# eblerjana/pangenie

Measured on AMD Instinct MI355X. Metric: genotyped variants/sec (whole node) at H haplotypes; HBM GB/s vs roofline, higher is better.
Workload: dtype f64

## Files before the change

include/pangenie_hmm.h:

```cpp
#ifndef PANGENIE_HMM_H
#define PANGENIE_HMM_H

#include <stddef.h>
#include <stdint.h>

#ifdef __cplusplus
extern "C" {
#endif

#define PG_OK 0
#define PG_ERR_INVALID (-1)
#define PG_ERR_NO_PATHS (-2)
#define PG_ERR_UNSUPPORTED (-3)
#define PG_ERR_DEVICE (-4)
#define PG_ERR_NOMEM (-5)

typedef struct pg_contig_batch {
    uint32_t n_variants;
    uint32_t n_paths;
    const uint64_t* variant_pos;
    const uint16_t* coverage;
    const uint32_t* kmer_off;
    const uint16_t* kmer_count;
    const uint32_t* allele_off;
    const uint16_t* allele_id;
    const uint8_t*  allele_flags;
    const uint16_t* allele_kmer_off;
    const uint32_t* allele_kmer_mask;
    const uint16_t* path_allele;
} pg_contig_batch;

typedef struct pg_hmm_params {
    long double effective_N;
    double recombrate;
    int32_t uniform;
    int32_t run_genotyping;
    int32_t run_phasing;
    int32_t reserved;
} pg_hmm_params;
#define PG_CALL_ANNOUNCED 1

typedef struct pg_contig_result {
    double*   lik;
    int32_t*  lik_exp;
    uint8_t*  kept;
    uint8_t*  allele_present;
    uint16_t* n_kmers;
    uint16_t* coverage;
    uint32_t  n_columns;
    uint32_t  reserved;
    uint16_t* haplotype_1;
    uint16_t* haplotype_2;
} pg_contig_result;

int pg_hmm_geno_offsets(const pg_contig_batch* batch, uint64_t* geno_off);

typedef struct pg_table pg_table;
pg_table* pg_table_create(uint16_t cov_min, uint16_t cov_max, uint16_t count_max,
                          long double regularization);
pg_table* pg_table_create_default(void);
int  pg_table_modify(pg_table* t, uint16_t coverage, uint16_t count,
                     long double p0, long double p1, long double p2);
int  pg_table_get(const pg_table* t, uint16_t coverage, uint16_t count,
                  long double out3[3]);
void pg_table_destroy(pg_table* t);

int pg_hmm_device_count(void);
const char* pg_hmm_version(void);
int pg_hmm_genotype_contig(const pg_contig_batch* batch, const pg_table* table,
                           const pg_hmm_params* params, int device,
                           pg_contig_result* out, char* err, size_t errlen);
void pg_hmm_announce(int device);
void pg_hmm_retract(int device);
int  pg_hmm_coalesce_stats(uint64_t out3[3]);

typedef struct pg_job pg_job;
pg_job* pg_job_create(int device, uint32_t n_contigs, const pg_contig_batch* batches,
                      const pg_table* table, const pg_hmm_params* params,
                      char* err, size_t errlen);
int  pg_job_run(pg_job* job, void* stream, char* err, size_t errlen);
int  pg_job_fetch(pg_job* job, uint32_t contig, pg_contig_result* out, char* err, size_t errlen);
int  pg_job_fetch_all(pg_job* job, pg_contig_result* outs, char* err, size_t errlen);
int  pg_job_device_results(pg_job* job, uint32_t contig, void** d_lik, uint64_t* n_lik,
                           void** d_lik_exp, uint64_t* n_variants);
#define PG_N_KERNEL_CLASSES 6
int  pg_job_kernel_ms(const pg_job* job, double ms[PG_N_KERNEL_CLASSES]);
const char* pg_job_kernel_name(int cls);
int  pg_job_profile_counters(pg_job* job, uint32_t contig, uint64_t out64[64]);
uint64_t pg_job_device_bytes(const pg_job* job);
int  pg_job_sweep_mode(const pg_job* job, uint32_t* chunk_cols);
uint32_t pg_job_triangle_chains(const pg_job* job);
double pg_job_index_ms(const pg_job* job);
size_t pg_job_plan(const pg_job* job, char* out, size_t len);
int pg_sparse_segment(uint32_t n_columns, uint32_t chunk_cols, uint32_t chunk, uint32_t role, uint32_t j, uint32_t out[3]);
int pg_sparse_stored_by_chain(uint32_t n_columns, uint32_t role, uint32_t column);
int pg_sparse_chunk_segment(uint32_t n_columns, uint32_t chunk_cols, uint32_t chunk, uint32_t role, uint32_t j, uint32_t out[3]);
int pg_sparse_chunk_stored_by_chain(uint32_t n_columns, uint32_t role, uint32_t column);
int pg_sparse_piece_range(uint32_t n_columns, uint32_t chunk_cols, uint32_t piece_chunks, uint32_t piece, uint32_t role, uint32_t out[2]);
double pg_job_viterbi_ms(const pg_job* job);
void pg_job_destroy(pg_job* job);

int  pg_job_panel_sizes(const pg_job* job, uint32_t contig, uint32_t* n_variants, uint32_t* n_paths,
                        uint64_t* sum_kmers, uint64_t* sum_alleles);
int  pg_job_fetch_panel(pg_job* job, uint32_t contig, uint32_t* kmer_off, uint16_t* kmer_count,
                        uint32_t* allele_off, uint16_t* allele_id, uint8_t* allele_flags,
                        uint16_t* allele_kmer_off, uint32_t* allele_kmer_mask, uint16_t* path_allele,
                        char* err, size_t errlen);

int  pg_job_new(int device, uint32_t n_contigs, const pg_contig_batch* batches,
                const pg_table* table, const pg_hmm_params* params,
                pg_job** out, char* err, size_t errlen);
uint32_t pg_job_n_chains(const pg_job* job);

typedef struct pg_sample_counts {
    const uint16_t* const* kmer_count;
    const uint16_t* const* coverage;
} pg_sample_counts;
int  pg_cohort_new(int device, uint32_t n_contigs, const pg_contig_batch* index,
                   uint32_t n_samples, const pg_sample_counts* samples,
                   const pg_table* table, const pg_hmm_params* params,
                   pg_job** out, char* err, size_t errlen);

int  pg_job_upload(pg_job* job, const pg_contig_batch* batches, const pg_sample_counts* samples,
                   char* err, size_t errlen);
int  pg_job_upload_run(pg_job* job, const pg_contig_batch* batches, const pg_sample_counts* samples, char* err, size_t errlen);
int  pg_job_upload_begin(pg_job* job, const pg_sample_counts* samples, char* err, size_t errlen);
int  pg_job_upload_end(pg_job* job, char* err, size_t errlen);
int  pg_job_host_seconds(const pg_job* job, double out4[4]);
int  pg_job_upload_bytes(const pg_job* job, uint64_t out2[2]);
int  pg_job_packed_results(pg_job* job, void** d_lik, void** d_lik_exp, uint64_t* n_lik_total);
void pg_hmm_release_cache(void);

typedef struct pg_comm pg_comm;
int  pg_comm_unique_id(uint8_t id128[128], char* err, size_t errlen);
int  pg_comm_init(const uint8_t id128[128], int world, int rank, int device,
                  pg_comm** out, char* err, size_t errlen);
int  pg_comm_init_all(int n_devices, const int* devices, pg_comm** out_comms, char* err, size_t errlen);
int  pg_comm_rank(const pg_comm* comm);
int  pg_comm_world(const pg_comm* comm);
void pg_comm_destroy(pg_comm* comm);
int  pg_hmm_gather(pg_comm* comm, pg_job* job, int root, const uint64_t* n_lik_per_rank,
                   void* d_lik_all, void* d_exp_all, char* err, size_t errlen);
int  pg_hmm_gather_all(int n_local, pg_comm* const* comms, pg_job* const* jobs, int root,
                       const uint64_t* n_lik_per_rank, void* d_lik_all, void* d_exp_all,
                       char* err, size_t errlen);
int  pg_hmm_gather_to_host(int n_local, pg_comm* const* comms, pg_job* const* jobs, int root,
                           const uint64_t* n_lik_per_rank, double* h_lik_all, int32_t* h_exp_all,
                           char* err, size_t errlen);

int pg_emission_table(const pg_contig_batch* batch, const pg_table* table, uint32_t v,
                      int device, long double* out_AxA, int32_t* all_zeros,
                      char* err, size_t errlen);
int pg_transition_probs(uint64_t from_pos, uint64_t to_pos, double recombrate,
                        uint32_t nr_paths, int uniform, long double effective_N,
                        int device, double out3[3], char* err, size_t errlen);

typedef struct pg_call {
    uint16_t allele_1, allele_2;
    uint16_t gq;
    uint16_t flags;
} pg_call;
#define PG_CALL_OK 0
#define PG_CALL_NONE 1
#define PG_CALL_NOT_UNIQUE 2
#define PG_CALL_DEFERRED 3
int  pg_job_calls(pg_job* job, char* err, size_t errlen);
int  pg_job_fetch_calls(pg_job* job, uint32_t chain, pg_call* out, char* err, size_t errlen);
int  pg_job_fetch_calls_all(pg_job* job, pg_call* const* outs, char* err, size_t errlen);
int  pg_job_device_calls(pg_job* job, uint32_t chain, void** d_calls, uint64_t* n);
double pg_job_calls_ms(const pg_job* job);
int  pg_calls_from_bins(int device, uint32_t n_variants, const uint32_t* allele_off, const uint16_t* allele_id,
                        const uint8_t* kept, const uint8_t* allele_present, const double* lik,
                        const int32_t* lik_exp, pg_call* out);

typedef struct pg_record_plan {
    uint32_t n_variants;
    uint32_t n_records;
    const uint32_t* rec_off;
    const uint32_t* map_off;
    const uint16_t* map;
    const uint16_t* n_alleles;
// ... 41 lines not shown
```

pangenie_amd/_lib.py:

```python
from __future__ import annotations

import ctypes as C

import numpy as np
import os
from pathlib import Path

ROOT = Path(__file__).resolve().parent.parent
HIP_LIB_PATH = ROOT / "pangenie_amd" / "csrc" / "libpangenie_hmm.so"

PG_OK = 0
PG_ERR_INVALID = -1
PG_ERR_NO_PATHS = -2
PG_ERR_UNSUPPORTED = -3
PG_ERR_DEVICE = -4
PG_ERR_NOMEM = -5
PG_N_KERNEL_CLASSES = 6

u8p = C.POINTER(C.c_uint8)
u16p = C.POINTER(C.c_uint16)
u32p = C.POINTER(C.c_uint32)
u64p = C.POINTER(C.c_uint64)
i32p = C.POINTER(C.c_int32)
f64p = C.POINTER(C.c_double)
# ... 42 lines not shown
    _fields_ = [
        ("lik", f64p),
        ("lik_exp", i32p),
        ("kept", u8p),
        ("allele_present", u8p),
        ("n_kmers", u16p),
        ("coverage", u16p),
        ("n_columns", C.c_uint32),
        ("reserved", C.c_uint32),
        ("haplotype_1", u16p),
        ("haplotype_2", u16p),
    ]


class PgSampleCounts(C.Structure):
    _fields_ = [
        ("kmer_count", C.POINTER(u16p)),
        ("coverage", C.POINTER(u16p)),
    ]


class PgGl(C.Structure):
    _fields_ = [("mant", C.c_int16), ("exp10", C.c_int16)]


PG_CALL_ANNOUNCED = 1


class HipExtensionMissing(RuntimeError):
    pass


_hip = None


def _bind_hip(lib):
    ld = C.c_longdouble
    lib.pg_hmm_geno_offsets.argtypes = [C.POINTER(PgContigBatch), u64p]
    lib.pg_hmm_geno_offsets.restype = C.c_int
    lib.pg_table_create.argtypes = [C.c_uint16, C.c_uint16, C.c_uint16, ld]
    lib.pg_table_create.restype = C.c_void_p
    lib.pg_table_create_default.argtypes = []
    lib.pg_table_create_default.restype = C.c_void_p
    lib.pg_table_modify.argtypes = [C.c_void_p, C.c_uint16, C.c_uint16, ld, ld, ld]
    lib.pg_table_modify.restype = C.c_int
    lib.pg_table_get.argtypes = [C.c_void_p, C.c_uint16, C.c_uint16, ldp]
    lib.pg_table_get.restype = C.c_int
    lib.pg_table_destroy.argtypes = [C.c_void_p]
    lib.pg_table_destroy.restype = None
    lib.pg_hmm_device_count.argtypes = []
    lib.pg_hmm_device_count.restype = C.c_int
    lib.pg_hmm_version.argtypes = []
    lib.pg_hmm_version.restype = C.c_char_p
    lib.pg_hmm_genotype_contig.argtypes = [
        C.POINTER(PgContigBatch), C.c_void_p, C.POINTER(PgHmmParams), C.c_int,
        C.POINTER(PgContigResult), C.c_char_p, C.c_size_t]
    lib.pg_hmm_genotype_contig.restype = C.c_int
    lib.pg_job_create.argtypes = [
        C.c_int, C.c_uint32, C.POINTER(PgContigBatch), C.c_void_p,
        C.POINTER(PgHmmParams), C.c_char_p, C.c_size_t]
    lib.pg_job_create.restype = C.c_void_p
    lib.pg_job_run.argtypes = [C.c_void_p, C.c_void_p, C.c_char_p, C.c_size_t]
    lib.pg_job_run.restype = C.c_int
    lib.pg_job_fetch.argtypes = [C.c_void_p, C.c_uint32, C.POINTER(PgContigResult),
                                 C.c_char_p, C.c_size_t]
    lib.pg_job_fetch.restype = C.c_int
    lib.pg_job_device_results.argtypes = [C.c_void_p, C.c_uint32, C.POINTER(C.c_void_p),
                                          u64p, C.POINTER(C.c_void_p), u64p]
    lib.pg_job_device_results.restype = C.c_int
    lib.pg_job_index_ms.argtypes = [C.c_void_p]
    lib.pg_job_index_ms.restype = C.c_double
    lib.pg_job_plan.argtypes = [C.c_void_p, C.c_char_p, C.c_size_t]
    lib.pg_job_plan.restype = C.c_size_t
    lib.pg_sparse_segment.argtypes = [C.c_uint32, C.c_uint32, C.c_uint32, C.c_uint32, C.c_uint32, u32p]
    lib.pg_sparse_segment.restype = C.c_int
    lib.pg_sparse_stored_by_chain.argtypes = [C.c_uint32, C.c_uint32, C.c_uint32]
    lib.pg_sparse_stored_by_chain.restype = C.c_int
    lib.pg_sparse_chunk_segment.argtypes = [C.c_uint32, C.c_uint32, C.c_uint32, C.c_uint32, C.c_uint32, u32p]
    lib.pg_sparse_chunk_segment.restype = C.c_int
    lib.pg_sparse_chunk_stored_by_chain.argtypes = [C.c_uint32, C.c_uint32, C.c_uint32]
    lib.pg_sparse_chunk_stored_by_chain.restype = C.c_int
    lib.pg_sparse_piece_range.argtypes = [C.c_uint32, C.c_uint32, C.c_uint32, C.c_uint32, C.c_uint32, u32p]
    lib.pg_sparse_piece_range.restype = C.c_int
    lib.pg_job_kernel_ms.argtypes = [C.c_void_p, f64p]
    lib.pg_job_kernel_ms.restype = C.c_int
    lib.pg_job_kernel_name.argtypes = [C.c_int]
    lib.pg_job_kernel_name.restype = C.c_char_p
    lib.pg_job_profile_counters.argtypes = [C.c_void_p, C.c_uint32, u64p]
    lib.pg_job_profile_counters.restype = C.c_int
    lib.pg_job_viterbi_ms.argtypes = [C.c_void_p]
    lib.pg_job_viterbi_ms.restype = C.c_double
    lib.pg_job_device_bytes.argtypes = [C.c_void_p]
    lib.pg_job_device_bytes.restype = C.c_uint64
    lib.pg_job_sweep_mode.argtypes = [C.c_void_p, C.POINTER(C.c_uint32)]
    lib.pg_job_sweep_mode.restype = C.c_int
    lib.pg_job_triangle_chains.argtypes = [C.c_void_p]
    lib.pg_job_triangle_chains.restype = C.c_uint32
    lib.pg_job_destroy.argtypes = [C.c_void_p]
    lib.pg_job_destroy.restype = None
    lib.pg_job_new.argtypes = [C.c_int, C.c_uint32, C.POINTER(PgContigBatch), C.c_void_p, C.POINTER(PgHmmParams),
                               C.POINTER(C.c_void_p), C.c_char_p, C.c_size_t]
    lib.pg_job_new.restype = C.c_int
    lib.pg_cohort_new.argtypes = [C.c_int, C.c_uint32, C.POINTER(PgContigBatch), C.c_uint32, C.POINTER(PgSampleCounts),
                                  C.c_void_p, C.POINTER(PgHmmParams), C.POINTER(C.c_void_p), C.c_char_p, C.c_size_t]
    lib.pg_cohort_new.restype = C.c_int
    lib.pg_job_n_chains.argtypes = [C.c_void_p]
    lib.pg_job_n_chains.restype = C.c_uint32
    lib.pg_job_upload.argtypes = [C.c_void_p, C.POINTER(PgContigBatch), C.POINTER(PgSampleCounts), C.c_char_p, C.c_size_t]
    lib.pg_job_upload.restype = C.c_int
    lib.pg_job_upload_run.argtypes = [C.c_void_p, C.POINTER(PgContigBatch), C.POINTER(PgSampleCounts), C.c_char_p, C.c_size_t]
    lib.pg_job_upload_run.restype = C.c_int
    lib.pg_job_upload_begin.argtypes = [C.c_void_p, C.POINTER(PgSampleCounts), C.c_char_p, C.c_size_t]
    lib.pg_job_upload_begin.restype = C.c_int
    lib.pg_job_upload_end.argtypes = [C.c_void_p, C.c_char_p, C.c_size_t]
    lib.pg_job_upload_end.restype = C.c_int
    lib.pg_job_host_seconds.argtypes = [C.c_void_p, f64p]
    lib.pg_job_host_seconds.restype = C.c_int
    lib.pg_job_upload_bytes.argtypes = [C.c_void_p, u64p]
    lib.pg_job_upload_bytes.restype = C.c_int
    lib.pg_job_packed_results.argtypes = [C.c_void_p, C.POINTER(C.c_void_p), C.POINTER(C.c_void_p), u64p]
    lib.pg_job_packed_results.restype = C.c_int
    lib.pg_hmm_release_cache.argtypes = []
    lib.pg_hmm_release_cache.restype = None
    lib.pg_comm_unique_id.argtypes = [u8p, C.c_char_p, C.c_size_t]
    lib.pg_comm_unique_id.restype = C.c_int
    lib.pg_comm_init.argtypes = [u8p, C.c_int, C.c_int, C.c_int, C.POINTER(C.c_void_p), C.c_char_p, C.c_size_t]
    lib.pg_comm_init.restype = C.c_int
    lib.pg_comm_init_all.argtypes = [C.c_int, C.POINTER(C.c_int), C.POINTER(C.c_void_p), C.c_char_p, C.c_size_t]
    lib.pg_comm_init_all.restype = C.c_int
    lib.pg_comm_rank.argtypes = [C.c_void_p]
    lib.pg_comm_rank.restype = C.c_int
    lib.pg_comm_world.argtypes = [C.c_void_p]
    lib.pg_comm_world.restype = C.c_int
    lib.pg_comm_destroy.argtypes = [C.c_void_p]
    lib.pg_comm_destroy.restype = None
    lib.pg_hmm_gather.argtypes = [C.c_void_p, C.c_void_p, C.c_int, u64p, C.c_void_p, C.c_void_p, C.c_char_p, C.c_size_t]
    lib.pg_hmm_gather.restype = C.c_int
    lib.pg_hmm_gather_all.argtypes = [C.c_int, C.POINTER(C.c_void_p), C.POINTER(C.c_void_p), C.c_int, u64p, C.c_void_p, C.c_void_p,
                                      C.c_char_p, C.c_size_t]
    lib.pg_hmm_gather_all.restype = C.c_int
    lib.pg_emission_table.argtypes = [C.POINTER(PgContigBatch), C.c_void_p, C.c_uint32, C.c_int,
                                      ldp, i32p, C.c_char_p, C.c_size_t]
    lib.pg_emission_table.restype = C.c_int
    lib.pg_transition_probs.argtypes = [C.c_uint64, C.c_uint64, C.c_double, C.c_uint32, C.c_int,
                                        ld, C.c_int, f64p, C.c_char_p, C.c_size_t]
    lib.pg_transition_probs.restype = C.c_int
    lib.pg_job_fetch_all.argtypes = [C.c_void_p, C.POINTER(PgContigResult), C.c_char_p, C.c_size_t]
    lib.pg_job_fetch_all.restype = C.c_int
    lib.pg_job_panel_sizes.argtypes = [C.c_void_p, C.c_uint32, C.POINTER(C.c_uint32), C.POINTER(C.c_uint32), u64p, u64p]
    lib.pg_job_panel_sizes.restype = C.c_int
    lib.pg_job_fetch_panel.argtypes = [C.c_void_p, C.c_uint32, u32p, u16p, u32p, u16p, u8p, u16p, u32p, u16p, C.c_char_p, C.c_size_t]
    lib.pg_job_fetch_panel.restype = C.c_int
    lib.pg_hmm_announce.argtypes = [C.c_int]
    lib.pg_hmm_announce.restype = None
    lib.pg_hmm_retract.argtypes = [C.c_int]
    lib.pg_hmm_retract.restype = None
    lib.pg_hmm_coalesce_stats.argtypes = [u64p]
    lib.pg_hmm_coalesce_stats.restype = C.c_int
    lib.pg_job_calls.argtypes = [C.c_void_p, C.c_char_p, C.c_size_t]
    lib.pg_job_calls.restype = C.c_int
    lib.pg_job_fetch_calls.argtypes = [C.c_void_p, C.c_uint32, C.c_void_p, C.c_char_p, C.c_size_t]
    lib.pg_job_fetch_calls.restype = C.c_int
    lib.pg_job_fetch_calls_all.argtypes = [C.c_void_p, C.POINTER(C.c_void_p), C.c_char_p, C.c_size_t]
    lib.pg_job_fetch_calls_all.restype = C.c_int
    lib.pg_job_device_calls.argtypes = [C.c_void_p, C.c_uint32, C.POINTER(C.c_void_p), u64p]
    lib.pg_job_device_calls.restype = C.c_int
    lib.pg_job_calls_ms.argtypes = [C.c_void_p]
    lib.pg_job_calls_ms.restype = C.c_double
    lib.pg_calls_from_bins.argtypes = [C.c_int, C.c_uint32, u32p, u16p, u8p, u8p, f64p, i32p, C.c_void_p]
    lib.pg_calls_from_bins.restype = C.c_int
    lib.pg_job_record_plan.argtypes = [C.c_void_p, C.c_uint32, C.c_void_p, C.c_char_p, C.c_size_t]
    lib.pg_job_record_plan.restype = C.c_int
    lib.pg_job_record_calls.argtypes = [C.c_void_p, C.c_char_p, C.c_size_t]
    lib.pg_job_record_calls.restype = C.c_int
    lib.pg_job_fetch_record_calls.argtypes = [C.c_void_p, C.c_uint32, C.c_void_p, C.c_char_p, C.c_size_t]
    lib.pg_job_fetch_record_calls.restype = C.c_int
    lib.pg_job_fetch_record_calls_all.argtypes = [C.c_void_p, C.POINTER(C.c_void_p), C.c_char_p, C.c_size_t]
    lib.pg_job_fetch_record_calls_all.restype = C.c_int
    lib.pg_job_device_record_calls.argtypes = [C.c_void_p, C.c_uint32, C.POINTER(C.c_void_p), u64p]
    lib.pg_job_device_record_calls.restype = C.c_int
    lib.pg_job_record_calls_ms.argtypes = [C.c_void_p]
    lib.pg_job_record_calls_ms.restype = C.c_double
    lib.pg_record_calls_from_bins.argtypes = [C.c_int, C.c_uint32, u32p, u16p, u8p, u8p, f64p, i32p, C.c_void_p, C.c_void_p]
    lib.pg_record_calls_from_bins.restype = C.c_int
    lib.pg_record_gl_offsets.argtypes = [C.c_void_p, u64p]
    lib.pg_record_gl_offsets.restype = C.c_int
    lib.pg_job_record_gl.argtypes = [C.c_void_p, C.c_char_p, C.c_size_t]
    lib.pg_job_record_gl.restype = C.c_int
    lib.pg_job_fetch_record_gl.argtypes = [C.c_void_p, C.c_uint32, C.c_void_p, C.c_char_p, C.c_size_t]
    lib.pg_job_fetch_record_gl.restype = C.c_int
    lib.pg_job_fetch_record_gl_all.argtypes = [C.c_void_p, C.POINTER(C.c_void_p), C.c_char_p, C.c_size_t]
    lib.pg_job_fetch_record_gl_all.restype = C.c_int
    lib.pg_job_device_record_gl.argtypes = [C.c_void_p, C.c_uint32, C.POINTER(C.c_void_p), u64p]
    lib.pg_job_device_record_gl.restype = C.c_int
    lib.pg_job_record_gl_ms.argtypes = [C.c_void_p]
    lib.pg_job_record_gl_ms.restype = C.c_double
    lib.pg_record_gl_from_bins.argtypes = [C.c_int, C.c_uint32, u32p, u16p, u8p, u8p, f64p, i32p, C.c_void_p, C.c_void_p]
    lib.pg_record_gl_from_bins.restype = C.c_int
    lib.pg_job_record_plan_strided.argtypes = [C.c_void_p, C.c_uint32, C.c_uint32, C.c_void_p, C.c_char_p, C.c_size_t]
    lib.pg_job_record_plan_strided.restype = C.c_int
    lib.pg_job_record_first.argtypes = [C.c_void_p, u64p, u64p, C.c_char_p, C.c_size_t]
    lib.pg_job_record_first.restype = C.c_int
    lib.pg_job_fetch_record_calls_packed.argtypes = [C.c_void_p, C.c_void_p, C.c_uint64, C.c_char_p, C.c_size_t]
    lib.pg_job_fetch_record_calls_packed.restype = C.c_int
    lib.pg_job_fetch_record_gl_packed.argtypes = [C.c_void_p, C.c_void_p, C.c_uint64, C.c_char_p, C.c_size_t]
    lib.pg_job_fetch_record_gl_packed.restype = C.c_int
    lib.pg_gl_from_values.argtypes = [C.c_int, C.c_uint64, u64p, i32p, C.c_void_p]
    lib.pg_gl_from_values.restype = C.c_int
    lib.pg_gl_text.argtypes = [PgGl, C.c_char_p, C.c_size_t]
    lib.pg_gl_text.restype = C.c_int
    return lib


HIP_ABI_SYMBOLS = [
    "pg_hmm_geno_offsets", "pg_table_create", "pg_table_create_default", "pg_table_modify",
    "pg_table_get", "pg_table_destroy", "pg_hmm_device_count", "pg_hmm_version",
    "pg_hmm_genotype_contig", "pg_job_create", "pg_job_run", "pg_job_fetch",
    "pg_job_device_results", "pg_job_profile_counters", "pg_job_kernel_ms", "pg_job_index_ms", "pg_job_plan", "pg_job_kernel_name", "pg_job_device_bytes", "pg_job_sweep_mode",
    "pg_job_destroy", "pg_emission_table", "pg_transition_probs",
    "pg_job_new", "pg_cohort_new", "pg_job_n_chains", "pg_job_upload", "pg_job_upload_run", "pg_job_upload_begin", "pg_job_upload_end", "pg_job_host_seconds", "pg_job_upload_bytes",
    "pg_job_packed_results", "pg_hmm_release_cache", "pg_job_triangle_chains", "pg_job_viterbi_ms",
    "pg_comm_unique_id", "pg_comm_init", "pg_comm_init_all", "pg_comm_rank", "pg_comm_world", "pg_comm_destroy",
    "pg_hmm_gather", "pg_hmm_gather_all", "pg_hmm_gather_to_host",
    "pg_hmm_announce", "pg_hmm_retract", "pg_hmm_coalesce_stats", "pg_job_fetch_all", "pg_job_panel_sizes", "pg_job_fetch_panel",
    "pg_job_calls", "pg_job_fetch_calls", "pg_job_fetch_calls_all", "pg_job_device_calls", "pg_job_calls_ms", "pg_calls_from_bins",
    "pg_job_record_plan", "pg_job_record_calls", "pg_job_fetch_record_calls", "pg_job_fetch_record_calls_all", "pg_job_device_record_calls",
    "pg_job_record_calls_ms", "pg_record_calls_from_bins",
    "pg_record_gl_offsets", "pg_job_record_gl", "pg_job_fetch_record_gl", "pg_job_fetch_record_gl_all", "pg_job_device_record_gl",
    "pg_job_record_gl_ms", "pg_record_gl_from_bins", "pg_gl_from_values", "pg_gl_text",
    "pg_job_record_plan_strided", "pg_job_record_first", "pg_job_fetch_record_calls_packed", "pg_job_fetch_record_gl_packed",
    "pg_sparse_segment", "pg_sparse_stored_by_chain", "pg_sparse_chunk_segment", "pg_sparse_chunk_stored_by_chain", "pg_sparse_piece_range",
]


def load_hip():
    global _hip
    if _hip is None:
        path = Path(os.environ.get("PANGENIE_HMM_LIB", HIP_LIB_PATH))
        if not path.exists():
            raise HipExtensionMissing(
                f"{path} is missing: run `python -c 'import __graft_entry__ as g; g.build()'` "
                "(hipcc --offload-arch=gfx950). There is no CPU fallback.")
        _hip = _bind_hip(C.CDLL(str(path), mode=os.RTLD_GLOBAL if hasattr(os, "RTLD_GLOBAL") else 0))
    return _hip
```

pangenie_amd/csrc/pg_device.h:

```cpp
#pragma once
#include <stddef.h>
#include <stdint.h>

#define PG_AMAX 5
#define PG_ESTRIDE (PG_AMAX + 1)
#define PG_ETAB (PG_ESTRIDE * PG_ESTRIDE)
#define PG_MAX_ALLELES_PER_VARIANT 256
#define PG_MAX_PATHS 1024
#define PG_PHANTOM 255

#define PG_REC_C0 0
#define PG_REC_C1 8
#define PG_REC_C2 16
#define PG_REC_KAPPA 24
#define PG_REC_VARIANT 32
#define PG_REC_EXP 36
#define PG_REC_NLOCAL 40
#define PG_REC_FLAGS 41
#define PG_REC_LOCAL_SLOT 48
#define PG_REC_BITS1 64
#define PG_REC_E 80
#define PG_REC_ALLELES (80 + 8 * PG_ETAB)
#define PG_REC_FLAG_ALLZERO 1
#define PG_REC_FLAG_WIDE 2
// ... 99 lines not shown
    uint8_t*  fwd_fallback;
    double*   scratch;
    uint32_t* sync;
    uint32_t  chunk_cols;
    uint32_t  col_stride;
    uint8_t*  wide;
    const uint32_t* wide_idx;
    uint8_t*  vpair;
    double*   frec;
    uint32_t  prep_fast;
    uint32_t  n_prep_m4, n_prep_w;
    uint32_t  n_prep_b;
    const uint32_t* prep_m4;
    const uint32_t* prep_w;
    const uint32_t* prep_b;
    uint32_t  lean;
    uint32_t  tri;
    uint32_t  leanx2;
    uint32_t  widef;
    uint32_t  small;
    uint32_t  leanx;
    uint32_t  cls4;
    uint32_t  smallx;
    uint32_t  split;
    const uint32_t* col_of;
    const unsigned char* ix_pd;
    const unsigned char* ix_rec;
    const unsigned char* ix_bin;
    unsigned char* cprec;
    uint32_t* ix_err;
    const uint32_t* ix_big;
    uint32_t n_ix_big;
    uint32_t sparse;
    uint32_t sparse2;
    uint32_t ckpt_slots;
    double*  ckpt;
    uint32_t* wcols;
    uint32_t* n_wcols;
    unsigned char* aux;
    const uint32_t* aux_idx;
    uint32_t  live;
    double*   xbuf;
    uint32_t* err;
    unsigned long long* prof;
    double*   vit_tq;
    uint16_t* vit_back;
    uint32_t* vit_best;
    uint16_t* hap1;
    uint16_t* hap2;
    double*   lik;
    int32_t*  lik_exp;
};

#define PG_LEAN_SPARSE 64u
#ifdef __HIP__
#define PG_HD __attribute__((host)) __attribute__((device))
#else
#define PG_HD
#endif
PG_HD inline uint32_t pg_sparse_segments(uint32_t C, uint32_t role) {
    const uint32_t mid = C / 2u;
    if (role == 0u) return mid ? (mid - 1u) / PG_LEAN_SPARSE : 0u;
    return C ? (C - 1u - mid) / PG_LEAN_SPARSE : 0u;
}
PG_HD inline uint32_t pg_sparse_checkpoint(uint32_t C, uint32_t role, uint32_t m) {
    const uint32_t mid = C / 2u;
    return role == 0u ? mid - 1u - m * PG_LEAN_SPARSE : mid + m * PG_LEAN_SPARSE;
}
PG_HD inline bool pg_sparse_stored(uint32_t C, uint32_t role, uint32_t c) {
    const uint32_t mid = C / 2u;
    if (role == 0u) return c >= mid || (mid - 1u - c) % PG_LEAN_SPARSE == 0u || c < (mid - 1u) % PG_LEAN_SPARSE;
    return c < mid || (c - mid) % PG_LEAN_SPARSE == 0u || c > mid + pg_sparse_segments(C, 1u) * PG_LEAN_SPARSE;
}
#define PG_PIECE_CHUNKS_DEFAULT 4u
PG_HD inline bool pg_sparse_piece(uint32_t C, uint32_t role, uint32_t piece_cols, uint32_t g, uint32_t out[2]) {
    const unsigned long long mid = C / 2u, half = role == 0u ? mid : C - mid;
    const unsigned long long d0 = (unsigned long long)g * piece_cols;
    if (piece_cols == 0u || piece_cols % PG_LEAN_SPARSE != 0u || d0 >= half) return false;
    const unsigned long long d1 = half - d0 > piece_cols ? d0 + piece_cols : half;
    if (role == 0u) { out[0] = (uint32_t)(mid - d1); out[1] = (uint32_t)(mid - 1u - d0); }
    else { out[0] = (uint32_t)(mid + d0); out[1] = (uint32_t)(mid + d1 - 1u); }
    return true;
}

PG_HD inline uint32_t pg_sparse2_slots(uint32_t V) { return (V / 2u + 1u) / PG_LEAN_SPARSE + 2u; }
PG_HD inline bool pg_sparse2_segment(uint32_t C, uint32_t role, unsigned long long m, uint32_t out[3]) {
    if (C < 2u) return false;
    const unsigned long long mid = C / 2u, d = m * PG_LEAN_SPARSE;
    if (role == 0u) {
        const unsigned long long ck = mid - 1u + d;
        if (ck + 1u >= C) return false;
        out[0] = (uint32_t)ck; out[1] = (uint32_t)ck + 1u; out[2] = (uint32_t)(C - 1u - ck > PG_LEAN_SPARSE ? ck + PG_LEAN_SPARSE : C - 1u);
    } else {
        if (d >= mid) return false;
        const unsigned long long ck = mid - d;
        out[0] = (uint32_t)ck; out[1] = (uint32_t)(ck > PG_LEAN_SPARSE ? ck - PG_LEAN_SPARSE : 0u); out[2] = (uint32_t)ck - 1u;
    }
    return true;
}
PG_HD inline bool pg_sparse2_stored(uint32_t C, uint32_t role, uint32_t c) {
    const uint32_t mid = C / 2u;
    if (C < 2u) return false;
    if (role == 0u) return c >= mid && c < C && (c - (mid - 1u)) % PG_LEAN_SPARSE == 0u;
    return c < mid && (mid - c) % PG_LEAN_SPARSE == 0u;
}

struct pg_job;
extern "C" {
__attribute__((visibility("hidden"))) int pgi_job_fill_begin(struct pg_job* job, uint32_t sample, int device, uint32_t n_contigs, const uint32_t* n_variants,
                                                            const uint32_t* const* kmer_off, void* stream, uint16_t** d_kmer_count, uint16_t** d_coverage,
                                                            char* err, size_t errlen);
__attribute__((visibility("hidden"))) int pgi_job_fill_end(struct pg_job* job, uint32_t sample, uint32_t n_contigs, const uint16_t* const* coverage, void* stream,
                                                          char* err, size_t errlen);
}
```

pangenie_amd/csrc/pg_job.h:

```cpp
#pragma once
#include <hip/hip_runtime_api.h>

#include <stdarg.h>
#include <stdint.h>
#include <stdio.h>

#include <chrono>
#include <memory>
#include <string>
#include <thread>
#include <vector>

#include "../../include/pangenie_hmm.h"
#include "pg_device.h"
#include "pg_launch.h"

namespace pgj __attribute__((visibility("hidden"))) {

inline void set_err(char* err, size_t errlen, const char* fmt, ...) {
    if (!err || errlen == 0) return;
    va_list ap;
    va_start(ap, fmt);
    vsnprintf(err, errlen, fmt, ap);
    va_end(ap);
// ... 67 lines not shown
}

struct OutputFamily {
    unsigned char* d = nullptr;
    std::vector<uint64_t> first;
    size_t o_desc = 0, o_wide = 0, o_stage = 0;
    uint32_t blocks = 0, wide = 0, max_bins = 0, stride = 0, slots = 0;
    bool dirty = true;
    bool formed = false;
    double ms = 0.0;
    void release() { if (d) hipFree(d); d = nullptr; }
};

}

struct pg_job {
    int device = 0;
    hipStream_t stream = nullptr;
    std::vector<pgj::IndexHost> index;
    std::vector<pgj::ChainHost> chains;
    uint32_t n_contigs = 0, n_samples = 1;
    bool cohort = false;
    DevContig* d_contigs = nullptr;
    unsigned char* arena = nullptr;
    size_t arena_bytes = 0;
    bool cache_arena = false;
    unsigned char* zero_base = nullptr;
    size_t zero_bytes = 0;
    uint32_t* d_small = nullptr;
    uint32_t n_small = 0;
    uint32_t* d_smallx = nullptr;
    uint32_t n_smallx = 0;
    bool smallx_phase2 = false;
    bool small_phase2 = false;
    double* d_dump = nullptr;
    uint32_t* d_ncols = nullptr;
    uint32_t* d_ixerr = nullptr;
    DevContig* d_reps = nullptr;
    unsigned char* ix_base = nullptr;
    size_t ix_bytes = 0;
    unsigned char* srec_base = nullptr;
    size_t srec_bytes = 0;
    bool any_split = false;
    uint32_t max_sb = 0, max_sm4 = 0, max_sw = 0;
    bool any_legacy_prep = false;
    hipEvent_t ev_ix[2];
    double index_ms = 0.0;
    std::string plan_text;
    std::vector<unsigned char> tab_p;
    size_t o_tab_p = 0;
    uint32_t* d_err = nullptr;
    double* d_lik = nullptr;
    int32_t* d_likexp = nullptr;
    uint64_t n_lik_total = 0;
    size_t o_tab_m = 0, o_tab_e = 0;
    std::vector<double> tab_m;
    std::vector<int32_t> tab_e;
    DevTable tab;
    uint32_t hp_mask = 0, max_v = 0;
    uint32_t max_wide = 0;
    uint32_t max_prep_w = 0, max_prep_m4 = 0;
    uint32_t bins_which = 0;
    uint32_t vit_bits = 0;
    hipEvent_t ev_vit[2];
    double vit_ms = 0.0;
    bool vit_tq_ready = false;
    hipEvent_t ev[PG_N_KERNEL_CLASSES + 1];
    bool events = false;
    double ms[PG_N_KERNEL_CLASSES] = {0, 0, 0, 0, 0, 0};
    double host_s[4] = {0, 0, 0, 0};
    uint64_t up_bytes[2] = {0, 0};
    pg_hmm_params params;
    bool ran = false;
    bool chunked = false;
    uint32_t chunk_cols = 0, n_chunks = 0;
    bool persist = false;
    uint32_t post_blocks = 0;
    bool sparse = false;
    bool sparse2 = false;
    std::vector<hipEvent_t> ev_chunk;
    uint32_t piece_chunks = 0, n_pieces = 1;
    uint32_t piece_refill_blocks = 0;
    std::vector<hipEvent_t> ev_piece;
    bool pipeline = false, pipeline_capable = false, late_pending = false;
    uint32_t nA = 0;
    std::vector<uint32_t> grp_order;
    DevContig* d_contigs_g = nullptr;
    DevContig* d_reps_g = nullptr;
    std::vector<std::thread> late_threads;
    std::vector<int> late_rc;
    hipEvent_t ev_late[2];
    bool ev_late_made = false;
    hipStream_t persist_checked = nullptr;
    bool persist_checked_any = false;
    uint32_t* d_handshake = nullptr;
    uint32_t persist_runs = 0, persist_fallbacks = 0;
    hipStream_t stream2 = nullptr;
    hipEvent_t ev_sweep[PG_SCRATCH_BUFS], ev_post[PG_SCRATCH_BUFS];
    bool events2 = false;
    size_t sample_lo = 0, sample_bytes = 0;
    unsigned char* staging = nullptr;
    bool staging_refused = false;
    unsigned char* alt_samples = nullptr;
    DevContig* d_contigs_alt = nullptr;
    DevContig* d_contigs_owned = nullptr;
    std::vector<DevContig> h_contigs;
    unsigned char* cur_samples = nullptr;
    hipStream_t copy_stream = nullptr;
    std::thread uploader;
    bool upload_pending = false;
    int upload_rc = PG_OK;
    std::string upload_err;
    std::vector<std::vector<uint16_t>> next_coverage;
    hipEvent_t ev_fill = nullptr;
    pgj::OutputFamily calls;
    std::vector<CallsDesc> calls_desc;
    hipEvent_t ev_calls[2];
    bool calls_events = false;
    std::vector<pgj::RecordPlanRef> rplans;
    bool rplan_ids_ok = false;
    pgj::OutputFamily rcalls;
    std::vector<RCallsDesc> rcalls_desc;
    pgj::OutputFamily rgl;
    std::vector<RGlDesc> rgl_desc;
};

namespace pgj __attribute__((visibility("hidden"))) {

inline void record_plans_changed(pg_job* job) {
    job->rcalls.dirty = true;
    job->rgl.dirty = true;
    job->rplan_ids_ok = false;
}

inline void join_late_threads(pg_job* job) {
    for (auto& t : job->late_threads) if (t.joinable()) t.join();
    job->late_threads.clear();
    job->late_pending = false;
}

inline uint32_t max_big_list(const pg_job* job) {
    uint32_t max_big = 0;
    for (const IndexHost& x : job->index) if (x.list_big.size() > max_big) max_big = (uint32_t)x.list_big.size();
    return max_big;
}

bool streams_concurrent(pg_job* job, hipStream_t s);

}
```

pangenie_amd/csrc/pg_kernels.hip:

```cpp
#include <hip/hip_runtime.h>
#include <math.h>
#include <stdint.h>
#include <stdlib.h>

#include <type_traits>

#include "pg_device.h"
#include "pg_devmath.h"
#include "pg_launch.h"

#define DEVI __device__ __forceinline__
typedef double v2f64 __attribute__((ext_vector_type(2)));
#include "pg_experiments.h"

template <int CTRL, int ROW_MASK, bool BOUND>
DEVI double dpp_f64(double v) {
    int lo = __double2loint(v), hi = __double2hiint(v);
    lo = __builtin_amdgcn_update_dpp(0, lo, CTRL, ROW_MASK, 0xF, BOUND);
    hi = __builtin_amdgcn_update_dpp(0, hi, CTRL, ROW_MASK, 0xF, BOUND);
    return __hiloint2double(hi, lo);
}

DEVI double readlane_f64(double v, int src_lane ) {
    int lo = __builtin_amdgcn_readlane(__double2loint(v), src_lane);
// ... 480 lines not shown
                v2f64* dst = (v2f64*)srec;
                dst[0] = ir[0]; dst[1] = ir[1];
                dst[2] = v2f64{E00, E01};
                dst[3] = v2f64{E11, __longlong_as_double((long long)packed)};
            }
        } else if (lane < 16u) {
            double out = val;
            if (lane == 15u) out = __longlong_as_double((long long)((unsigned long long)(uint32_t)X | ((unsigned long long)fl << 32)));
            ((double*)srec)[lane] = out;
        }
        if (precise && lane < 16u) {
            ((double*)(dc.cprec + (size_t)col * PG_CPREC_BYTES))[lane] = !mine ? 0.0 : (all_zeros ? 0.5 : pm);
            ((int*)(dc.cprec + (size_t)col * PG_CPREC_BYTES + 128u))[lane] = !mine ? 0 : (all_zeros ? 1 : pe);
        }
        return;
    }
    if (lane < PG_ETAB) s_E[wave][lane] = 0.0;
    wave_sync_lds();
    if (mine) {
        double val;
        if (all_zeros) val = 1.0;
        else val = (pm > 0.0) ? ldexp(pm, pe - X) : pm;
        s_E[wave][la * PG_ESTRIDE + lb] = val;
        s_E[wave][lb * PG_ESTRIDE + la] = val;
        const uint32_t pn = dc.pair_n, NP = (pn * (pn + 1) / 2 + 1u) & ~1u;
        unsigned char* vp = dc.vpair + (size_t)v * (NP * 12u);
        const uint32_t pi = tri_n(la, lb, pn);
        ((double*)vp)[pi] = all_zeros ? 0.5 : pm;
        ((int*)(vp + (size_t)NP * 8u))[pi] = all_zeros ? 1 : pe;
    }
    wave_sync_lds();
    if (lane < PG_ETAB) ((double*)(rec + PG_REC_E))[lane] = s_E[wave][lane];
    if (lane < 4) ((double*)rec)[lane] = 0.0;
    if (lane == 0) {
        *(uint32_t*)(rec + PG_REC_VARIANT) = v;
        *(int32_t*)(rec + PG_REC_EXP) = X;
        rec[PG_REC_NLOCAL] = (unsigned char)n_local;
        rec[PG_REC_FLAGS] = all_zeros ? PG_REC_FLAG_ALLZERO : 0;
        rec[PG_REC_FLAGS + 1] = 0; rec[PG_REC_FLAGS + 2] = 0;
        *(uint32_t*)(rec + PG_REC_WIDE_IDX) = PG_WIDE_NONE;
        uint16_t* ls = (uint16_t*)(rec + PG_REC_LOCAL_SLOT);
        uint32_t l = 0;
        for (uint32_t s = 0; s < A && l < 8; ++s)
            if (slot_present(pres, s)) ls[l++] = (uint16_t)s;
        for (; l < 8; ++l) ls[l] = 0;
        *(uint32_t*)(rec + PG_REC_AUX) = dc.aux_idx ? dc.aux_idx[v] : PG_WIDE_NONE;
    }
}
__global__ __launch_bounds__(256) void k_prep(const DevContig* __restrict__ contigs, DevTable tab) {
    const DevContig& dc = contigs[blockIdx.y];
    if (dc.prep_fast == 1u || dc.split) return;
#pragma unroll 1
    for (uint32_t r = 0; r < (uint32_t)PG_VREP; ++r) {
        prep_unit<false>(dc, tab, blockIdx.x * (uint32_t)PG_VREP + r);
        wave_sync_lds();
    }
}
__global__ __launch_bounds__(256) void k_prep_s_w(const DevContig* __restrict__ contigs, DevTable tab) {
    const DevContig& dc = contigs[blockIdx.y];
    if (!dc.split || !dc.prep_w) return;
#pragma unroll 1
    for (uint32_t r = 0; r < (uint32_t)PG_VREP; ++r) {
        prep_unit<true>(dc, tab, blockIdx.x * (uint32_t)PG_VREP + r);
        wave_sync_lds();
    }
}




template <int CTRL>
DEVI void dpp_mul_step(double& m, int& e) {
    const int lo = __builtin_amdgcn_update_dpp(0, __double2loint(m), CTRL, 0xF, 0xF, false);
    const int hi = __builtin_amdgcn_update_dpp(0x3FF00000, __double2hiint(m), CTRL, 0xF, 0xF, false);
    const int oe = __builtin_amdgcn_update_dpp(0, e, CTRL, 0xF, 0xF, false);
    m *= __hiloint2double(hi, lo);
    e += oe;
}
DEVI double row_last_f64(double v) {
    return __longlong_as_double(__builtin_amdgcn_update_dpp(__double_as_longlong(v), __double_as_longlong(v), 0x15F, 0xF, 0xF, true));
}
DEVI int row_last_i32(int v) { return __builtin_amdgcn_update_dpp(v, v, 0x15F, 0xF, 0xF, true); }

DEVI void prep_bi_unit(const DevContig& dc, const DevTable& tab, uint32_t unit) {
    const uint32_t lane = threadIdx.x & 63u, grp = lane >> 4, l = lane & 15u;
    const uint32_t nobj = dc.prep_b ? dc.n_prep_b : dc.V;
    const uint32_t pos = unit * 16u + (threadIdx.x >> 6) * 4u + grp;
    if (unit * 16u + (threadIdx.x >> 6) * 4u >= nobj) return;
    bool live = pos < nobj;
    const uint32_t v = dc.prep_b ? dc.prep_b[live ? pos : nobj - 1u] : pos;
    const uint32_t vv = live ? v : dc.V - 1u;
    const uint32_t H = dc.H, HP = dc.HP;
    const uint32_t a0 = dc.allele_off[vv];
    const bool mine = dc.prep_fast != 2u || (dc.allele_off[vv + 1] - a0 == 2u && dc.kmer_off[vv + 1] - dc.kmer_off[vv] <= 32u);
    live = live && mine;
    const uint32_t a1 = mine ? a0 + 1u : a0;
    const uint16_t id0 = dc.allele_id[a0], id1 = dc.allele_id[a1];
    const bool u0 = dc.allele_flags[a0] & 1, u1 = dc.allele_flags[a1] & 1;
    uint32_t slot[4];
    bool bad = false, nonref = false, has0 = false, has1 = false;
    unsigned long long ones = 0;
#pragma unroll
    for (int i = 0; i < 4; ++i) {
        const uint32_t p = 16u * (uint32_t)i + l;
        const bool inb = live && p < H;
        const uint16_t a = inb ? dc.path_allele[(size_t)vv * H + p] : (uint16_t)0;
        const bool s1 = inb && a == id1, s0 = inb && !s1 && a == id0;
        slot[i] = s1 ? 1u : 0u;
        bad = bad || (inb && !s1 && !s0);
        has0 = has0 || s0;
        has1 = has1 || s1;
        nonref = nonref || ((s1 || s0) && a != 0 && !(s1 ? u1 : u0));
        const unsigned long long b = __ballot(s1);
        ones |= ((b >> (16u * grp)) & 0xFFFFull) << (16u * (uint32_t)i);
    }
    const uint32_t sh16 = 16u * grp;
    const bool any_bad = ((__ballot(bad) >> sh16) & 0xFFFFull) != 0, kept = ((__ballot(nonref) >> sh16) & 0xFFFFull) != 0;
    has0 = ((__ballot(has0) >> sh16) & 0xFFFFull) != 0;
    has1 = ((__ballot(has1) >> sh16) & 0xFFFFull) != 0;
    if (!live) return;
    if (any_bad) {
        if (l == 0) { atomicOr(dc.err, PG_DEVERR_ALLELE_NOT_FOUND); dc.kept[v] = 0; }
        return;
    }
    if (l == 0) { dc.allele_present[a0] = has0 ? 1 : 0; dc.kept[v] = kept ? 1 : 0; }
    if (l == 1) dc.allele_present[a0 + 1] = has1 ? 1 : 0;
    if (!kept) return;
    const uint32_t n_local = (has0 ? 1u : 0u) + (has1 ? 1u : 0u);
    const uint32_t loc1 = has0 ? 1u : 0u;
    __shared__ unsigned char s_rec[4][4][448] __attribute__((aligned(16)));
    unsigned char* rec = s_rec[threadIdx.x >> 6][grp];
#pragma unroll
    for (int i = 0; i < 4; ++i) {
        const uint32_t p = 16u * (uint32_t)i + l;
        if (p < HP) rec[PG_REC_ALLELES + p] = (unsigned char)(p < H ? (slot[i] ? loc1 : 0u) : (uint32_t)PG_PHANTOM);
    }
    for (uint32_t pad = PG_REC_ALLELES + HP + l; pad < dc.RB; pad += 16u) rec[pad] = 0;
    const uint32_t k0 = dc.kmer_off[v], K = dc.kmer_off[v + 1] - k0, cov = dc.cov[v];
    const uint32_t off0 = dc.allele_koff[a0], mask0 = dc.allele_kmask[a0], off1 = dc.allele_koff[a0 + 1], mask1 = dc.allele_kmask[a0 + 1];
    double pm[3] = {1.0, 1.0, 1.0};
    int pe[3] = {0, 0, 0};
#pragma unroll
    for (int j = 0; j < 2; ++j) {
        const uint32_t k = 16u * (uint32_t)j + l;
        if (k < K) {
            double m[3]; int e[3];
            cn_lookup(tab, cov, dc.kmer_count[k0 + k], m, e);
            const uint32_t on0 = kmer_on(off0, mask0, k), on1 = kmer_on(off1, mask1, k);
            auto factor = [&](uint32_t c, bool ua, bool ub, double& fm, int& fe) {
                const double mc = c == 0 ? m[0] : (c == 1 ? m[1] : m[2]);
                const int ec = c == 0 ? e[0] : (c == 1 ? e[1] : e[2]);
                if (ua && ub) mix3(m, e, 1.0 / 3.0, fm, fe);
                else if (ua || ub) {
                    const double m2 = c == 0 ? m[1] : m[2];
                    const int e2 = c == 0 ? e[1] : e[2];
                    mix2(mc, ec, m2, e2, 0.5, fm, fe);
                } else { fm = mc; fe = ec; }
            };
            double fm; int fe;
            factor(2u * on0, u0, u0, fm, fe); pm[0] *= fm; pe[0] += fe;
            factor(on0 + on1, u0, u1, fm, fe); pm[1] *= fm; pe[1] += fe;
            factor(2u * on1, u1, u1, fm, fe); pm[2] *= fm; pe[2] += fe;
        }
    }
#pragma unroll
    for (int q = 0; q < 3; ++q) {
        dpp_mul_step<0x111>(pm[q], pe[q]);
        dpp_mul_step<0x112>(pm[q], pe[q]);
        dpp_mul_step<0x114>(pm[q], pe[q]);
        dpp_mul_step<0x118>(pm[q], pe[q]);
        pm[q] = row_last_f64(pm[q]);
        pe[q] = row_last_i32(pe[q]);
        double mm; int ee;
// ... 271 lines not shown
}
__global__ __launch_bounds__(256) void k_prep_m4(const DevContig* __restrict__ contigs, DevTable tab) {
    const DevContig& dc = contigs[blockIdx.y];
    if (!dc.prep_m4 || dc.split) return;
#pragma unroll 1
    for (uint32_t r = 0; r < (uint32_t)PG_VREP; ++r) prep_m4_unit<false>(dc, tab, blockIdx.x * (uint32_t)PG_VREP + r);
}
__global__ __launch_bounds__(256) void k_prep_s_m4(const DevContig* __restrict__ contigs, DevTable tab) {
    const DevContig& dc = contigs[blockIdx.y];
    if (!dc.prep_m4 || dc.split != 2u) return;
#pragma unroll 1
    for (uint32_t r = 0; r < (uint32_t)PG_VREP; ++r) prep_m4_unit<true>(dc, tab, blockIdx.x * (uint32_t)PG_VREP + r);
}

__global__ __launch_bounds__(64) void k_emission_single(const DevContig* __restrict__ contigs, DevTable tab,
                                                        uint32_t v, double* out_m, int* out_e) {
    __shared__ double s_m[64 * 3];
    __shared__ int s_e[64 * 3];
    const DevContig& dc = contigs[0];
    const uint32_t lane = threadIdx.x;
    const uint32_t A = dc.allele_off[v + 1] - dc.allele_off[v];
    const uint32_t P = A * (A + 1) / 2;
    for (uint32_t base = 0; base < P; base += 64) {
        const bool active = base + lane < P;
        uint32_t s1 = 0, s2 = 0;
        if (active) decode_pair(base + lane, A, s1, s2);
        double pm; int pe;
        emission_pair_products(dc, tab, v, lane, active, s1, s2, s_m, s_e, pm, pe);
        if (active) {
            out_m[s1 * A + s2] = pm; out_e[s1 * A + s2] = pe;
            out_m[s2 * A + s1] = pm; out_e[s2 * A + s1] = pe;
        }
    }
}

__global__ __launch_bounds__(1024) void k_compact(const DevContig* __restrict__ contigs) {
    __shared__ uint32_t s_cnt[1024];
    const DevContig& dc = contigs[blockIdx.x];
    const uint32_t tid = threadIdx.x, V = dc.V;
    const uint32_t chunk = (V + 1023u) / 1024u;
    const uint32_t lo = tid * chunk < V ? tid * chunk : V;
    const uint32_t hi = lo + chunk < V ? lo + chunk : V;
    uint32_t cnt = 0;
    for (uint32_t v = lo; v < hi; ++v) cnt += dc.kept[v] ? 1u : 0u;
    s_cnt[tid] = cnt;
    __syncthreads();
    for (uint32_t off = 1; off < 1024; off <<= 1) {
        uint32_t add = tid >= off ? s_cnt[tid - off] : 0u;
        __syncthreads();
        s_cnt[tid] += add;
        __syncthreads();
    }
    uint32_t pos = s_cnt[tid] - cnt;
    uint32_t* col_of = const_cast<uint32_t*>(dc.col_of);
    for (uint32_t v = lo; v < hi; ++v) {
        if (col_of) col_of[v] = dc.kept[v] ? pos : PG_COL_NONE;
        if (dc.kept[v]) dc.col_variant[pos++] = v;
    }
    if (tid == 1023) *dc.n_cols = s_cnt[1023];
}

DEVI void transition_consts(double d, uint32_t H, int uniform, double& c0, double& c1, double& c2, double& kappa) {
    if (uniform) { c0 = 0.0; c1 = 0.0; c2 = 1.0; }
    else {
        const double x = d / (double)H;
        const double r = exp(-x);
        const double q = one_minus_exp_neg_like_reference(x) / (double)H;
        c0 = r * r; c1 = q * r; c2 = q * q;
    }
    const double h = (double)H;
    kappa = c0 + 2.0 * h * c1 + h * h * c2;
}

__global__ __launch_bounds__(64) void k_transition_single(double d, uint32_t H, int uniform, double* out3) {
    if (threadIdx.x == 0) {
        transition_probs_f64(d, H, uniform, out3[0], out3[1], out3[2]);
    }
}

DEVI bool compact_records_only(const DevContig& dc, uint32_t C) {
    return ((dc.tri == 2u || dc.small == 2u || dc.smallx == 2u) && C >= 2u) || (dc.lean && dc.tri == 0u && dc.chunk_cols > 0u);
}

DEVI void records_unit(const DevContig& dc, uint32_t unit) {
    const uint32_t wave = threadIdx.x >> 6, lane = threadIdx.x & 63;
    const uint32_t C = *dc.n_cols;
    if (dc.split) return;
    if (compact_records_only(dc, C) && !dc.smallx) {
        const uint32_t c = unit * 256u + threadIdx.x;
        if (c >= C) return;
        const uint32_t v = dc.col_variant[c];
        const uint64_t* src = (const uint64_t*)(dc.vrec + (size_t)v * dc.RB);
        double c0 = 0.0, c1 = 0.0, c2 = 0.0, kappa = 0.0;
        if (c > 0) {
            const double d = (double)(dc.pos[v] - dc.pos[dc.col_variant[c - 1]]) * dc.dist_scale;
            transition_consts(d, dc.H, dc.uniform, c0, c1, c2, kappa);
        }
        const uint64_t* E = src + PG_REC_E / 8;
        typedef double f64x2 __attribute__((ext_vector_type(2)));
        f64x2* out = (f64x2*)(dc.frec + (size_t)c * 8);
        out[0] = f64x2{c0, c1};
        out[1] = f64x2{c2, kappa};
        out[2] = f64x2{__longlong_as_double((long long)E[0]), __longlong_as_double((long long)E[1])};
        out[3] = f64x2{__longlong_as_double((long long)E[PG_ESTRIDE + 1]), __longlong_as_double((long long)src[PG_REC_BITS1 / 8])};
        return;
    }
    __shared__ double s_c[4][64][4];
    __shared__ uint32_t s_v[4][64];
    const uint32_t cbase = (unit * 4u + wave) * 64u;
    if (cbase >= C) return;
    {
        const uint32_t c = cbase + lane;
        double c0 = 0.0, c1 = 0.0, c2 = 0.0, kappa = 0.0;
        uint32_t v = 0;
        if (c < C) {
            v = dc.col_variant[c];
            if (c > 0) {
                const double d = (double)(dc.pos[v] - dc.pos[dc.col_variant[c - 1]]) * dc.dist_scale;
                transition_consts(d, dc.H, dc.uniform, c0, c1, c2, kappa);
            }
        }
        s_c[wave][lane][0] = c0; s_c[wave][lane][1] = c1; s_c[wave][lane][2] = c2; s_c[wave][lane][3] = kappa;
        s_v[wave][lane] = v;
        if (c < C && dc.wcols && (dc.vrec[(size_t)v * dc.RB + PG_REC_FLAGS] & PG_REC_FLAG_WIDE)) dc.wcols[atomicAdd(dc.n_wcols, 1u)] = c;
    }
    wave_sync_lds();
    const uint32_t n = C - cbase < 64u ? C - cbase : 64u;
    const uint32_t ppr = dc.RB / 16u, inv = (uint32_t)((0x100000000ull + ppr - 1u) / ppr);
    typedef double f64x2 __attribute__((ext_vector_type(2)));
    f64x2* dst = (f64x2*)(dc.colrec + (size_t)cbase * dc.RB);
    if (!compact_records_only(dc, C))
    for (uint32_t p = lane; p < n * ppr; p += 64u) {
        const uint32_t q = __umulhi(p, inv), w = p - q * ppr;
        const uint32_t v = s_v[wave][q];
        f64x2 val = ((const f64x2*)(dc.vrec + (size_t)v * dc.RB))[w];
        if (w < 2u) val = f64x2{s_c[wave][q][2u * w], s_c[wave][q][2u * w + 1u]};
        dst[p] = val;
    }
    if (dc.smallx) {
        f64x2* xd = (f64x2*)((unsigned char*)dc.frec + (size_t)cbase * 192u);
        for (uint32_t p = lane; p < n * 12u; p += 64u) {
            const uint32_t q = p / 12u, w = p - q * 12u;
            const unsigned char* src = dc.vrec + (size_t)s_v[wave][q] * dc.RB;
            const uint32_t nlf = (uint32_t)src[PG_REC_NLOCAL] | ((uint32_t)src[PG_REC_FLAGS] << 8);
            const bool widec = (nlf & 0x200u) != 0u;
            f64x2 val = f64x2{0.0, 0.0};
            if (w < 8u) {
                if (widec) { if (w == 0u) val = *(const f64x2*)(src + PG_REC_ALLELES); }
                else {
                    auto entry = [&](uint32_t e) {
                        if (e >= 15u) return 0.0;
                        const uint32_t a = (e >= 5u ? 1u : 0u) + (e >= 9u ? 1u : 0u) + (e >= 12u ? 1u : 0u) + (e >= 14u ? 1u : 0u);
                        const uint32_t b = e - (a * (uint32_t)PG_AMAX - a * (a - 1u) / 2u) + a;
                        return ((const double*)(src + PG_REC_E))[a * PG_ESTRIDE + b];
                    };
                    val = f64x2{entry(2u * w), entry(2u * w + 1u)};
                }
            } else if (w == 9u) val = f64x2{s_c[wave][q][0], s_c[wave][q][1]};
            else if (w == 10u) val = f64x2{s_c[wave][q][2], s_c[wave][q][3]};
            else {
                uint4 u;
                if (w == 8u) u = uint4{nlf, *(const uint32_t*)(src + PG_REC_WIDE_IDX), *(const uint32_t*)(src + PG_REC_AUX), 0u};
                else {
                    u = *(const uint4*)(src + PG_REC_ALLELES);
                    auto f = [&](uint32_t x) {
                        uint32_t r = 0;
#pragma unroll
                        for (int b = 0; b < 4; ++b) {
                            const uint32_t a = (x >> (8 * b)) & 0xFFu;
                            r |= ((a < (uint32_t)PG_AMAX && !widec) ? (a + 1u) * (uint32_t)(PG_ESTRIDE * 8) : 0u) << (8 * b);
                        }
                        return r;
                    };
                    u = uint4{f(u.x), f(u.y), f(u.z), f(u.w)};
                }
                val = *(const f64x2*)&u;
            }
            xd[p] = val;
        }
    }
    if (dc.lean || dc.small) {
        for (uint32_t p = lane; p < n * 8u; p += 64u) {
            const uint32_t q = p >> 3, f = p & 7u;
            const uint64_t* src = (const uint64_t*)(dc.vrec + (size_t)s_v[wave][q] * dc.RB);
            uint64_t val;
            if (f < 4u) val = (uint64_t)__double_as_longlong(s_c[wave][q][f]);
            else if (f == 4u) val = src[PG_REC_E / 8];
            else if (f == 5u) val = src[PG_REC_E / 8 + 1];
            else if (f == 6u) val = src[PG_REC_E / 8 + PG_ESTRIDE + 1];
// ... 4962 lines not shown
}

__global__ __launch_bounds__(256) void k_bins_wide(const DevContig* __restrict__ contigs) {
    __shared__ double s_bins[4][PG_AMAX * (PG_AMAX + 1) / 2];
    __shared__ double s_wide[4][PG_WIDE_LDS_BINS];
    const DevContig& dc = contigs[blockIdx.y];
    const uint32_t C = *dc.n_cols;
    if (!(bins_x(dc, C) || dc.widef) || !dc.wcols) return;
    const uint32_t wave = threadIdx.x >> 6, lane = threadIdx.x & 63u;
    const uint32_t id = blockIdx.x * 4u + wave;
    if (id >= *dc.n_wcols) return;
    const uint32_t c = (uint32_t)__builtin_amdgcn_readfirstlane((int)dc.wcols[id]);
    const unsigned char* rec = dc.vrec + (size_t)dc.col_variant[c] * dc.RB;
    const uint32_t ax = (uint32_t)__builtin_amdgcn_readfirstlane((int)*(const uint32_t*)(rec + PG_REC_AUX));
    const size_t colsz = (size_t)dc.HP * dc.HP;
    const double* mine = (const double*)(dc.aux + (size_t)ax * 16u);
    const double* stored = dc.fwd + (size_t)c * (dc.tri ? (size_t)dc.col_stride : colsz);
    const uint32_t st = dc.tri ? 1u : 0u;
    if (c >= C / 2) post_ab(dc, C, c, mine, stored, lane, s_bins[wave], s_wide[wave], st << 1);
    else post_ab(dc, C, c, stored, mine, lane, s_bins[wave], s_wide[wave], st);
}

#include "pg_split.h"

#define PG_MAX_DEVICES 64
static bool lds_attr_pending(bool (&done)[PG_MAX_DEVICES]) {
    int dev = -1;
    if (hipGetDevice(&dev) != hipSuccess || dev < 0 || dev >= PG_MAX_DEVICES) return true;
    if (done[dev]) return false;
    done[dev] = true;
    return true;
}
template <int HP, int R, int VBUF, bool KEEPW, int PHASE>
static void launch_one(const DevContig* d_contigs, uint32_t n_contigs, uint32_t chunk, hipStream_t s) {
    using Cfg = ChainCfg<HP, R, sweep_has_loader<HP, PHASE>()>;
    size_t dyn = (Cfg::LOADER && PHASE == 2) ? (size_t)kRingSlots * HP * HP * 8 : 0;
    if (!Cfg::LOADER && PHASE == 2) dyn = (size_t)(Cfg::PARK / 2) * 16 * Cfg::T;
    if (HP == 64 && dyn > 0) {
        if (dyn < kTriRingB) dyn = kTriRingB;
    }
    auto kern = k_sweep<HP, R, VBUF, KEEPW, PHASE>;
    static bool attr_done[PG_MAX_DEVICES];
    if (dyn > 0 && lds_attr_pending(attr_done))
        (void)hipFuncSetAttribute((const void*)kern, hipFuncAttributeMaxDynamicSharedMemorySize, (int)dyn);
    hipLaunchKernelGGL(kern, dim3(n_contigs, 2), dim3(Cfg::TT), dyn, s, d_contigs, chunk);
}
template <int PHASE>
static void launch_sweep(const DevContig* d_contigs, uint32_t n_contigs, uint32_t hp_mask, uint32_t chunk, hipStream_t s) {
    if (hp_mask & PG_SWEEP_HP16) launch_one<16, 4, 1, true, PHASE>(d_contigs, n_contigs, chunk, s);
#ifndef PG_HP32_ROWS
#define PG_HP32_ROWS 8
#endif
    if (hp_mask & PG_SWEEP_HP32) launch_one<32, PG_HP32_ROWS, 1, true, PHASE>(d_contigs, n_contigs, chunk, s);
    if (hp_mask & PG_SWEEP_HP64) launch_one<64, 16, 1, true, PHASE>(d_contigs, n_contigs, chunk, s);
    if constexpr (PHASE == 1) {
        if (hp_mask & PG_SWEEP_TRI1)
            hipLaunchKernelGGL(k_sweep_tri1, dim3(n_contigs, 2), dim3(ChainCfg<64, 16, sweep_has_loader<64, 1>()>::TT), 0, s, d_contigs);
        if (hp_mask & PG_SWEEP_LEANX_TRI)
            hipLaunchKernelGGL(k_sweep_leanx_tri, dim3(n_contigs, 2), dim3(LxCfg<64>::T), 0, s, d_contigs);
        if (hp_mask & PG_SWEEP_LEANX_TRIW)
            hipLaunchKernelGGL(k_sweep_leanx_triw, dim3(n_contigs, 2), dim3(LxCfg<64>::T), 0, s, d_contigs);
    }
    if (hp_mask & PG_SWEEP_HP128) launch_one<128, 32, 1, false, PHASE>(d_contigs, n_contigs, chunk, s);
    if constexpr (PHASE == 2) {
        if (hp_mask & PG_SWEEP_LEAN2) hipLaunchKernelGGL((k_sweep_lean2<16>), dim3(n_contigs, 2), dim3(256), 0, s, d_contigs);
        if (hp_mask & PG_SWEEP_LEANX2) hipLaunchKernelGGL(k_sweep_leanx2, dim3(n_contigs, 2), dim3(256), 0, s, d_contigs);
    }
    if constexpr (PHASE != 2) {
        if (hp_mask & PG_SWEEP_LEAN) {
            if (PHASE == 1 && (hp_mask & PG_SWEEP_TRI))
                hipLaunchKernelGGL((k_sweep_lean_tri<PHASE, 16>), dim3(n_contigs, 2), dim3(256), 0, s, d_contigs, chunk);
            else hipLaunchKernelGGL((k_sweep_lean<PHASE, 16, false>), dim3(n_contigs, 2), dim3(256), 0, s, d_contigs, chunk);
        }
        if (hp_mask & PG_SWEEP_LEANX128)
            hipLaunchKernelGGL((k_sweep_leanx<PHASE, 128>), dim3(n_contigs, 2), dim3(LxCfg<128>::T), 0, s, d_contigs, chunk);
        if (hp_mask & PG_SWEEP_LEANX64)
            hipLaunchKernelGGL((k_sweep_leanx<PHASE, 64>), dim3(n_contigs, 2), dim3(LxCfg<64>::T), 0, s, d_contigs, chunk);
        const bool from64 = hp_mask & PG_SWEEP_GENERIC64;
        if (hp_mask & (PG_SWEEP_GENERIC | PG_SWEEP_GENERIC64))
            hipLaunchKernelGGL(k_sweep_generic<PHASE>, dim3(n_contigs, 2), dim3(PG_GEN_THREADS), 0, s, d_contigs, chunk,
                               from64 ? 64u : 256u);
    }
}
extern "C" {

void pgk_launch_prep(const DevContig* d_contigs, uint32_t n_contigs, uint32_t max_v, uint32_t max_w, uint32_t max_m4, DevTable tab, hipStream_t s) {
    dim3 grid((max_w + 4 * PG_VREP - 1) / (4 * PG_VREP), n_contigs);
    if (max_w) hipLaunchKernelGGL(k_prep, grid, dim3(256), 0, s, d_contigs, tab);
    dim3 grid16((max_v + 16 * PG_VREP - 1) / (16 * PG_VREP), n_contigs);
    hipLaunchKernelGGL(k_prep_bi, grid16, dim3(256), 0, s, d_contigs, tab);
    dim3 gridm((max_m4 + 16 * PG_VREP - 1) / (16 * PG_VREP), n_contigs);
    if (max_m4) hipLaunchKernelGGL(k_prep_m4, gridm, dim3(256), 0, s, d_contigs, tab);
}
void pgk_launch_compact(const DevContig* d_contigs, uint32_t n_contigs, hipStream_t s) {
    hipLaunchKernelGGL(k_compact, dim3(n_contigs), dim3(1024), 0, s, d_contigs);
}
void pgk_launch_index(const DevContig* d_reps, uint32_t n_index, uint32_t max_v, uint32_t max_big, int any_split, hipStream_t s) {
    if (max_v == 0 || n_index == 0) return;
    hipLaunchKernelGGL(k_index_scan_t, dim3((max_v + 255u) / 256u, n_index), dim3(256), 0, s, d_reps);
    if (max_big) hipLaunchKernelGGL(k_index_scan, dim3((max_big + 3u) / 4u, n_index), dim3(256), 0, s, d_reps);
    hipLaunchKernelGGL(k_compact, dim3(n_index), dim3(1024), 0, s, d_reps);
    if (any_split) {
        hipLaunchKernelGGL(k_index_cols_t, dim3((max_v + 255u) / 256u, n_index), dim3(256), 0, s, d_reps);
        if (max_big) hipLaunchKernelGGL(k_index_cols, dim3((max_big + 3u) / 4u, n_index), dim3(256), 0, s, d_reps);
    }
}
void pgk_launch_prep_split(const DevContig* d_contigs, uint32_t n_contigs, uint32_t max_b, uint32_t max_m4, uint32_t max_w, DevTable tab, hipStream_t s) {
    if (max_b) hipLaunchKernelGGL(k_prep_s_bi, dim3((max_b + 255u) / 256u, n_contigs), dim3(256), 0, s, d_contigs, tab);
    if (max_m4) hipLaunchKernelGGL(k_prep_s_m4, dim3((max_m4 + 16 * PG_VREP - 1) / (16 * PG_VREP), n_contigs), dim3(256), 0, s, d_contigs, tab);
    if (max_w) hipLaunchKernelGGL(k_prep_s_w, dim3((max_w + 4 * PG_VREP - 1) / (4 * PG_VREP), n_contigs), dim3(256), 0, s, d_contigs, tab);
}
void pgk_launch_records(const DevContig* d_contigs, uint32_t n_contigs, uint32_t max_v, hipStream_t s) {
    dim3 grid((max_v + 255) / 256, n_contigs);
    hipLaunchKernelGGL(k_records, grid, dim3(256), 0, s, d_contigs);
}
void pgk_launch_bins(const DevContig* d_contigs, uint32_t n_contigs, uint32_t max_v, uint32_t which, uint32_t max_wide, hipStream_t s) {
    const bool full = which & PG_BINS_FULL;
    dim3 grid(full ? (max_v + 3) / 4 : 1u, n_contigs);
    hipLaunchKernelGGL(k_bins, grid, dim3(256), 0, s, d_contigs);
    dim3 grid256((max_v + 255) / 256, n_contigs), grid16((max_v + 15u) / 16u, n_contigs);
    if (which & PG_BINS_LEAN2) hipLaunchKernelGGL(k_bins_lean2, grid256, dim3(256), 0, s, d_contigs);
    if (which & PG_BINS_THIN) hipLaunchKernelGGL(k_bins_thin, grid256, dim3(256), 0, s, d_contigs);
    if (which & PG_BINS_X) hipLaunchKernelGGL(k_bins_x, grid256, dim3(256), 0, s, d_contigs);
    if ((which & PG_BINS_WIDE) && max_wide)
        hipLaunchKernelGGL(k_bins_wide, dim3((max_wide + 3u) / 4u, n_contigs), dim3(256), 0, s, d_contigs);
    if (which & PG_BINS_S) hipLaunchKernelGGL(k_bins_s, grid256, dim3(256), 0, s, d_contigs);
    if ((which & PG_BINS_WIDE_S) && max_wide)
        hipLaunchKernelGGL(k_bins_wide_s, dim3((max_wide + 3u) / 4u, n_contigs), dim3(256), 0, s, d_contigs);
    if (which & PG_BINS_Q) hipLaunchKernelGGL(k_bins_q, grid16, dim3(256), 0, s, d_contigs);
}
void pgk_launch_sweep(const DevContig* d_contigs, uint32_t n_contigs, uint32_t hp_mask, int phase, hipStream_t s) {
    if (phase == 1) launch_sweep<1>(d_contigs, n_contigs, hp_mask, 0, s);
    else launch_sweep<2>(d_contigs, n_contigs, hp_mask, 0, s);
}
void pgk_launch_sweep_piece(const DevContig* d_contigs, uint32_t n_contigs, uint32_t piece_chunks, uint32_t piece, hipStream_t s) {
    hipLaunchKernelGGL((k_sweep_lean<1, 16, false>), dim3(n_contigs, 2), dim3(256), 0, s, d_contigs, (piece_chunks << 16) | piece);
}
void pgk_launch_sweep_chunk(const DevContig* d_contigs, uint32_t n_contigs, uint32_t hp_mask, uint32_t chunk, hipStream_t s) {
    launch_sweep<3>(d_contigs, n_contigs, hp_mask, chunk, s);
}
void pgk_launch_sweep_small(const DevContig* d_contigs, const uint32_t* d_ids, uint32_t n_ids, int phase, uint32_t chunk, double* d_dump, hipStream_t s) {
    if (n_ids == 0) return;
    const dim3 grid((n_ids + 3u) / 4u, 2);
    if (phase == 1) hipLaunchKernelGGL(k_sweep_small16<1>, grid, dim3(64), 0, s, d_contigs, d_ids, n_ids, chunk, d_dump);
    else if (phase == 2) hipLaunchKernelGGL(k_sweep_small16<2>, grid, dim3(64), 0, s, d_contigs, d_ids, n_ids, chunk, d_dump);
    else hipLaunchKernelGGL(k_sweep_small16<3>, grid, dim3(64), 0, s, d_contigs, d_ids, n_ids, chunk, d_dump);
}
void pgk_launch_sweep_smallx(const DevContig* d_contigs, const uint32_t* d_ids, uint32_t n_ids, int phase, uint32_t chunk, double* d_dump, hipStream_t s) {
    if (n_ids == 0) return;
    const dim3 grid((n_ids + 3u) / 4u, 2);
    if (phase == 1) hipLaunchKernelGGL(k_sweep_small16x<1>, grid, dim3(64), 0, s, d_contigs, d_ids, n_ids, chunk, d_dump);
    else if (phase == 2) hipLaunchKernelGGL(k_sweep_small16x<2>, grid, dim3(64), 0, s, d_contigs, d_ids, n_ids, chunk, d_dump);
    else hipLaunchKernelGGL(k_sweep_small16x<3>, grid, dim3(64), 0, s, d_contigs, d_ids, n_ids, chunk, d_dump);
}
uint32_t pgk_post_blocks(uint32_t n_contigs, uint32_t chunk_cols, uint32_t* cus_out) {
    static int cus[PG_MAX_DEVICES];
    int dev = 0;
    if (hipGetDevice(&dev) != hipSuccess || dev < 0 || dev >= PG_MAX_DEVICES) dev = 0;
    if (cus[dev] == 0) {
        hipDeviceProp_t prop;
        cus[dev] = (hipGetDeviceProperties(&prop, dev) == hipSuccess && prop.multiProcessorCount > 0) ? prop.multiProcessorCount : 256;
    }
    if (cus_out) *cus_out = (uint32_t)cus[dev];
    const int idle = cus[dev] - 2 * (int)n_contigs;
    const uint32_t cap = idle > (int)n_contigs ? (uint32_t)(idle / (int)n_contigs) : 1u;
    uint32_t bx = (2u * chunk_cols + PG_POST_WAVES - 1u) / PG_POST_WAVES;
    if (bx > cap) bx = cap;
    if (const char* e = getenv("PG_POST_BLOCKS")) { const long v = strtol(e, nullptr, 0); if (v >= 1 && (uint32_t)v < bx) bx = (uint32_t)v; }
    return bx ? bx : 1u;
}
void pgk_launch_refill(const DevContig* d_contigs, uint32_t n_contigs, uint32_t chunk_cols, uint32_t chunk, int phase2, uint32_t max_blocks, hipStream_t s) {
    static bool attr_done[PG_MAX_DEVICES];
    if (lds_attr_pending(attr_done))
        (void)hipFuncSetAttribute((const void*)k_refill_lean<16>, hipFuncAttributeMaxDynamicSharedMemorySize, PG_REFILL_PLACEMENT_LDS);
    uint32_t cus = 0;
    (void)pgk_post_blocks(n_contigs, chunk_cols, &cus);
    const uint32_t q = chunk_cols / PG_LEAN_SPARSE;
    uint32_t blocks = cus > 2u * n_contigs + n_contigs ? cus - 2u * n_contigs : n_contigs;
    if (const char* e = getenv("PG_REFILL_BLOCKS")) { const long v = strtol(e, nullptr, 0); if (v >= 1 && (uint32_t)v < blocks) blocks = (uint32_t)v; }
    if (max_blocks && blocks > max_blocks) blocks = max_blocks;
    if (blocks > 2u * q * n_contigs) blocks = 2u * q * n_contigs;
    if (blocks == 0u) return;
    hipLaunchKernelGGL((k_refill_lean<16>), dim3(blocks), dim3(256), PG_REFILL_PLACEMENT_LDS, s, d_contigs, n_contigs, chunk, q, phase2 ? 1u : 0u);
}
void pgk_launch_post(const DevContig* d_contigs, uint32_t n_contigs, uint32_t chunk_cols, uint32_t chunk, hipStream_t s) {
    static bool attr_done[PG_MAX_DEVICES];
    if (lds_attr_pending(attr_done))
        (void)hipFuncSetAttribute((const void*)k_post, hipFuncAttributeMaxDynamicSharedMemorySize, PG_POST_PLACEMENT_LDS);
    const uint32_t per_chain = pgk_post_blocks(n_contigs, chunk_cols, nullptr);
    if (n_contigs <= 64u && getenv("PG_POST_FIXED") == nullptr) {
        uint32_t cus = 0;
        (void)pgk_post_blocks(n_contigs, chunk_cols, &cus);
        uint32_t total = cus > 2u * n_contigs + n_contigs ? cus - 2u * n_contigs : n_contigs;
        if (const char* e = getenv("PG_POST_BLOCKS")) { const long v = strtol(e, nullptr, 0); if (v >= 1) total = std::min<uint32_t>(total, (uint32_t)v * n_contigs); }
        const uint32_t most = ((2u * chunk_cols + PG_POST_WAVES - 1u) / PG_POST_WAVES) * n_contigs;
        if (total > most) total = most;
        hipLaunchKernelGGL(k_post, dim3(total, 1), dim3(64 * PG_POST_WAVES), PG_POST_PLACEMENT_LDS, s, d_contigs, chunk, n_contigs);
// ... 41 lines not shown
```

pangenie_amd/csrc/pg_launch.h:

```cpp
#pragma once
#include <hip/hip_runtime_api.h>
#include <stdint.h>

#include "pg_device.h"

enum : uint32_t {
    PG_SWEEP_HP16 = 1u,
    PG_SWEEP_HP32 = 2u,
    PG_SWEEP_HP64 = 4u,
    PG_SWEEP_HP128 = 8u,
    PG_SWEEP_GENERIC = 16u,
    PG_SWEEP_GENERIC64 = 32u,
    PG_SWEEP_LEAN = 64u,
    PG_SWEEP_TRI = 128u,
    PG_SWEEP_LEAN2 = 256u,
    PG_SWEEP_LEANX128 = 512u,
    PG_SWEEP_LEANX64 = 1024u,
    PG_SWEEP_TRI1 = 2048u,
    PG_SWEEP_LEANX_TRI = 4096u,
    PG_SWEEP_LEANX2 = 8192u,
    PG_SWEEP_LEANX_TRIW = 16384u,
};

enum : uint32_t {
    PG_BINS_FULL = 1u,
    PG_BINS_LEAN2 = 2u,
    PG_BINS_THIN = 4u,
    PG_BINS_X = 8u,
    PG_BINS_WIDE = 16u,
    PG_BINS_S = 32u,
    PG_BINS_WIDE_S = 64u,
    PG_BINS_Q = 128u,
};

struct CallsDesc {
    uint32_t blk0, V;
    uint32_t chain, pad;
    void* out;
};

struct RecPlanDev {
    const uint32_t* rec_var;
    const uint32_t* map_off;
    const uint16_t* map;
    const uint32_t* vcf_off;
    const uint16_t* vcf_index;
};
struct RCallsDesc {
    uint32_t blk0, R;
    uint32_t chain, pad;
    void* out;
    RecPlanDev plan;
};

struct RGlDesc {
    uint32_t blk0, R;
    uint32_t chain, pad;
    void* out;
    const uint64_t* gl_off;
    RecPlanDev plan;
};

extern "C" {
void pgk_launch_rgl(const DevContig* d_contigs, const RGlDesc* d_desc, uint32_t n_desc, uint32_t n_blocks, const void* d_wide, uint32_t n_wide,
                    void* d_stage, uint32_t max_bins, uint32_t stride, uint32_t n_slots, hipStream_t s);
void pgk_launch_gl_values(const uint64_t* d_m, const int32_t* d_e, void* d_out, uint32_t n, hipStream_t s);
void pgk_launch_rcalls(const DevContig* d_contigs, const RCallsDesc* d_desc, uint32_t n_desc, uint32_t n_blocks, const void* d_wide, uint32_t n_wide,
                       void* d_stage, uint32_t max_bins, uint32_t stride, uint32_t n_slots, const uint64_t* d_thr_m, const int32_t* d_thr_e, hipStream_t s);
void pgk_launch_rplan_ids(const DevContig* d_contigs, const RCallsDesc* d_desc, uint32_t n_desc, uint32_t n_blocks, void* d_hit, hipStream_t s);
void pgk_launch_calls(const DevContig* d_contigs, const CallsDesc* d_desc, uint32_t n_desc, uint32_t n_blocks, const void* d_wide, uint32_t n_wide,
                      const uint64_t* d_thr_m, const int32_t* d_thr_e, hipStream_t s);
uint32_t pgk_calls_block(void);
void pgk_launch_prep(const DevContig* d_contigs, uint32_t n_contigs, uint32_t max_v, uint32_t max_w, uint32_t max_m4, DevTable tab, hipStream_t s);
void pgk_launch_compact(const DevContig* d_contigs, uint32_t n_contigs, hipStream_t s);
void pgk_launch_index(const DevContig* d_reps, uint32_t n_index, uint32_t max_v, uint32_t max_big, int any_split, hipStream_t s);
void pgk_launch_prep_split(const DevContig* d_contigs, uint32_t n_contigs, uint32_t max_b, uint32_t max_m4, uint32_t max_w, DevTable tab, hipStream_t s);
void pgk_launch_records(const DevContig* d_contigs, uint32_t n_contigs, uint32_t max_v, hipStream_t s);
void pgk_launch_bins(const DevContig* d_contigs, uint32_t n_contigs, uint32_t max_v, uint32_t which, uint32_t max_wide, hipStream_t s);
void pgk_launch_sweep(const DevContig* d_contigs, uint32_t n_contigs, uint32_t hp_mask, int phase, hipStream_t s);
void pgk_launch_sweep_piece(const DevContig* d_contigs, uint32_t n_contigs, uint32_t piece_chunks, uint32_t piece, hipStream_t s);
void pgk_launch_sweep_chunk(const DevContig* d_contigs, uint32_t n_contigs, uint32_t hp_mask, uint32_t chunk, hipStream_t s);
void pgk_launch_sweep_small(const DevContig* d_contigs, const uint32_t* d_ids, uint32_t n_ids, int phase, uint32_t chunk, double* d_dump, hipStream_t s);
void pgk_launch_sweep_smallx(const DevContig* d_contigs, const uint32_t* d_ids, uint32_t n_ids, int phase, uint32_t chunk, double* d_dump, hipStream_t s);
uint32_t pgk_post_blocks(uint32_t n_contigs, uint32_t chunk_cols, uint32_t* cus_out);
void pgk_launch_post(const DevContig* d_contigs, uint32_t n_contigs, uint32_t chunk_cols, uint32_t chunk, hipStream_t s);
void pgk_launch_refill(const DevContig* d_contigs, uint32_t n_contigs, uint32_t chunk_cols, uint32_t chunk, int phase2, uint32_t max_blocks, hipStream_t s);
void pgk_launch_stream_handshake(uint32_t* d_words, hipStream_t s, hipStream_t s2);
void pgk_launch_phase2_persistent(const DevContig* d_contigs, uint32_t n_contigs, uint32_t post_blocks, hipStream_t s, hipStream_t s2);
void pgk_launch_emission_single(const DevContig* d_contig, DevTable tab, uint32_t v, double* out_m, int* out_e, hipStream_t s);
void pgk_launch_transition_single(double d, uint32_t H, int uniform, double* out3, hipStream_t s);
uint32_t pgk_threads_for_hp(uint32_t hp);
void pgk_launch_viterbi(const DevContig* d_contigs, uint32_t n, uint32_t max_v, uint32_t hp_bits, hipStream_t s);
}
```

pangenie_amd/csrc/pg_shim.cpp:

```cpp
#include <hip/hip_runtime_api.h>

#include <math.h>
#include <stdarg.h>
#include <stdio.h>
#include <stdlib.h>
#include <string.h>

#include <algorithm>
#include <atomic>
#include <chrono>
#include <condition_variable>
#include <map>
#include <memory>
#include <mutex>
#include <string>
#include <thread>
#include <vector>

#include "../../include/pangenie_hmm.h"
#include "pg_device.h"
#include "pg_job.h"
#include "pg_launch.h"

using namespace pgj;
// ... 188 lines not shown
    bool take(int device, size_t need, unsigned char** ptr, size_t* bytes) {
        std::lock_guard<std::mutex> lock(mu);
        int best = -1;
        for (size_t i = 0; i < free_list.size(); ++i)
            if (free_list[i].device == device && free_list[i].bytes >= need && (best < 0 || free_list[i].bytes < free_list[(size_t)best].bytes)) best = (int)i;
        if (best < 0) return false;
        *ptr = free_list[(size_t)best].ptr; *bytes = free_list[(size_t)best].bytes;
        free_list.erase(free_list.begin() + best);
        return true;
    }
    void put(int device, unsigned char* ptr, size_t bytes) {
        std::vector<Entry> drop;
        {
            std::lock_guard<std::mutex> lock(mu);
            free_list.push_back({device, ptr, bytes});
            size_t total = 0;
            for (const Entry& e : free_list) if (e.device == device) total += e.bytes;
            const size_t lim = limit(device);
            while (total > lim) {
                long k = -1;
                for (size_t i = 0; i < free_list.size(); ++i)
                    if (free_list[i].device == device && (k < 0 || free_list[i].bytes < free_list[(size_t)k].bytes)) k = (long)i;
                if (k < 0) break;
                total -= free_list[(size_t)k].bytes;
                drop.push_back(free_list[(size_t)k]);
                free_list.erase(free_list.begin() + k);
            }
        }
        for (const Entry& e : drop)
            if (hipSetDevice(e.device) == hipSuccess) hipFree(e.ptr);
        if (!drop.empty()) hipSetDevice(device);
    }
    void clear() {
        std::vector<Entry> all;
        { std::lock_guard<std::mutex> lock(mu); all.swap(free_list); }
        for (const Entry& e : all)
            if (hipSetDevice(e.device) == hipSuccess) hipFree(e.ptr);
    }
} g_pool;

struct PinnedPool {
    static constexpr size_t kBytes = (size_t)16 << 20;
    std::mutex mu;
    std::vector<unsigned char*> free_list;
    unsigned char* get() {
        { std::lock_guard<std::mutex> l(mu); if (!free_list.empty()) { unsigned char* p = free_list.back(); free_list.pop_back(); return p; } }
        void* p = nullptr;
        if (hipHostMalloc(&p, kBytes, hipHostMallocDefault) != hipSuccess) { (void)hipGetLastError(); return nullptr; }
        return (unsigned char*)p;
    }
    void put(unsigned char* p) { if (p) { std::lock_guard<std::mutex> l(mu); free_list.push_back(p); } }
    void clear() { std::lock_guard<std::mutex> l(mu); for (unsigned char* p : free_list) hipHostFree(p); free_list.clear(); }
} g_pinned;

}

extern "C" void pg_job_destroy(pg_job* job) {
    if (!job) return;
    hipSetDevice(job->device);
    if (job->uploader.joinable()) job->uploader.join();
    for (auto& t : job->late_threads) if (t.joinable()) t.join();
    if (job->ev_late_made) { hipEventDestroy(job->ev_late[0]); hipEventDestroy(job->ev_late[1]); }
    if (job->copy_stream) { hipStreamSynchronize(job->copy_stream); hipStreamDestroy(job->copy_stream); }
    if (job->ev_fill) hipEventDestroy(job->ev_fill);
    if (job->calls_events) { hipEventDestroy(job->ev_calls[0]); hipEventDestroy(job->ev_calls[1]); }
    if (job->staging) hipHostFree(job->staging);
    if (job->alt_samples) hipFree(job->alt_samples);
    if (job->d_contigs_owned) hipFree(job->d_contigs_owned);
    if (job->stream) hipStreamSynchronize(job->stream);
    if (job->stream2) hipStreamSynchronize(job->stream2);
    job->calls.release();
    job->rcalls.release();
    job->rgl.release();
    job->rplans.clear();
    if (job->events) {
        for (auto& e : job->ev) hipEventDestroy(e);
        for (auto& e : job->ev_vit) hipEventDestroy(e);
        for (auto& e : job->ev_ix) hipEventDestroy(e);
    }
    if (job->events2)
        for (int q = 0; q < (int)PG_SCRATCH_BUFS; ++q) { hipEventDestroy(job->ev_sweep[q]); hipEventDestroy(job->ev_post[q]); }
    for (hipEvent_t e : job->ev_chunk) hipEventDestroy(e);
    for (hipEvent_t e : job->ev_piece) hipEventDestroy(e);
    if (job->arena) {
        if (job->cache_arena) g_pool.put(job->device, job->arena, job->arena_bytes);
        else hipFree(job->arena);
    }
    if (job->stream2) hipStreamDestroy(job->stream2);
    if (job->stream) hipStreamDestroy(job->stream);
    delete job;
}

extern "C" void pg_hmm_release_cache(void) {
    int cur = -1;
    const bool have = hipGetDevice(&cur) == hipSuccess;
    g_pool.clear();
    g_pinned.clear();
    if (have) hipSetDevice(cur);
}

namespace {

struct ChainSpec { uint32_t index; const uint16_t* kmer_count; const uint16_t* coverage; };

int sample_upload(pg_job* job, const std::vector<ChainSpec>& specs, unsigned char* dev_base, hipStream_t stream,
                  std::vector<std::vector<uint16_t>>* cov_out, uint64_t* bytes, char* err, size_t errlen) {
    const size_t n = job->chains.size();
    if (!job->staging && !job->staging_refused) {
        hipError_t he = hipHostMalloc((void**)&job->staging, job->sample_bytes ? job->sample_bytes : 8, hipHostMallocDefault);
        if (he != hipSuccess) { (void)hipGetLastError(); job->staging = nullptr; job->staging_refused = true; }
    }
    if (!job->staging) {
        const size_t lo0 = job->sample_lo;
        for (size_t c = 0; c < n; ++c) {
            ChainHost& ch = job->chains[c];
            const IndexHost& x = job->index[ch.index];
            if (x.V == 0) continue;
            HIP_TRY(hipMemcpyAsync(dev_base + (ch.o_cov - lo0), specs[c].coverage, (size_t)x.V * 2, hipMemcpyHostToDevice, stream));
            if (x.sumK) HIP_TRY(hipMemcpyAsync(dev_base + (ch.o_kcnt - lo0), specs[c].kmer_count, (size_t)x.sumK * 2, hipMemcpyHostToDevice, stream));
            if (bytes) *bytes += (uint64_t)x.V * 2 + (uint64_t)x.sumK * 2;
            if (cov_out) (*cov_out)[c].assign(specs[c].coverage, specs[c].coverage + x.V);
        }
        HIP_TRY(hipStreamSynchronize(stream));
        return PG_OK;
    }
    size_t pieces = n / 64;
    const unsigned hw = std::thread::hardware_concurrency();
    const size_t cap = hw ? (hw > 32 ? 16 : (hw + 1) / 2) : 4;
    if (pieces > cap) pieces = cap;
    if (pieces < 1) pieces = 1;
    std::vector<int> rcs(pieces, (int)hipSuccess);
    std::vector<uint64_t> moved(pieces, 0);
    const size_t lo0 = job->sample_lo;
    auto work = [&](size_t k) {
        if (hipSetDevice(job->device) != hipSuccess) { rcs[k] = (int)hipErrorInvalidDevice; return; }
        const size_t c0 = n * k / pieces, c1 = n * (k + 1) / pieces;
        if (c0 >= c1) return;
        for (size_t c = c0; c < c1; ++c) {
            ChainHost& ch = job->chains[c];
            const IndexHost& x = job->index[ch.index];
            if (x.V == 0) continue;
            memcpy(job->staging + (ch.o_cov - lo0), specs[c].coverage, (size_t)x.V * 2);
            if (x.sumK) memcpy(job->staging + (ch.o_kcnt - lo0), specs[c].kmer_count, (size_t)x.sumK * 2);
            moved[k] += (uint64_t)x.V * 2 + (uint64_t)x.sumK * 2;
            if (cov_out) (*cov_out)[c].assign(specs[c].coverage, specs[c].coverage + x.V);
        }
        const size_t b0 = job->chains[c0].o_cov - lo0;
        const size_t b1 = c1 < n ? job->chains[c1].o_cov - lo0 : job->sample_bytes;
        if (b1 > b0) rcs[k] = (int)hipMemcpyAsync(dev_base + b0, job->staging + b0, b1 - b0, hipMemcpyHostToDevice, stream);
    };
    std::vector<std::thread> th;
    for (size_t k = 1; k < pieces; ++k) th.emplace_back(work, k);
    work(0);
    for (auto& t : th) t.join();
    for (size_t k = 0; k < pieces; ++k) {
        if (rcs[k] != (int)hipSuccess) { set_err(err, errlen, "sample upload: %s", hipGetErrorString((hipError_t)rcs[k])); return PG_ERR_DEVICE; }
        if (bytes) *bytes += moved[k];
    }
    HIP_TRY(hipStreamSynchronize(stream));
    return PG_OK;
}

int upload_inputs(pg_job* job, const pg_contig_batch* batches, const std::vector<ChainSpec>& specs, bool with_index,
                  char* err, size_t errlen) {
    const double t0 = now_s();
    unsigned char* A = job->arena;
    hipStream_t s = job->stream;
    uint64_t bi = 0, bs = 0;
    struct Copy { void* dst; const void* src; size_t bytes; };
    struct LateGuard { pg_job* job; bool armed; ~LateGuard() { if (armed) join_late_threads(job); } } late_guard{job, false};
    std::vector<Copy> copies, late_copies;
    if (with_index && job->pipeline && !streams_concurrent(job, s)) job->pipeline = false;
    const bool pipe = with_index && job->pipeline;
    job->pipeline = false;
    std::vector<char> late(job->chains.size(), 0);
    if (pipe) for (size_t k = job->nA; k < job->grp_order.size(); ++k) late[job->grp_order[k]] = 1;
    bool cur_late = false;
#define UP(off, src, bytes, acc)                                                                              \
    do {                                                                                                      \
        if ((bytes) > 0) {                                                                                    \
            (cur_late ? late_copies : copies).push_back({(void*)(A + (off)), (const void*)(src), (size_t)(bytes)});   \
            acc += (uint64_t)(bytes);                                                                         \
        }                                                                                                     \
    } while (0)
    if (with_index) {
        record_plans_changed(job);
        for (size_t i = 0; i < job->index.size(); ++i) {
            const pg_contig_batch& b = batches[i];
            IndexHost& x = job->index[i];
            if (x.V == 0) continue;
            cur_late = pipe && late[i];
            UP(x.o_pos, b.variant_pos, (size_t)x.V * 8, bi);
            if (job->params.run_phasing) { x.pos.assign(b.variant_pos, b.variant_pos + x.V); job->vit_tq_ready = false; }
            UP(x.o_koff, b.kmer_off, ((size_t)x.V + 1) * 4, bi);
            UP(x.o_aoff, b.allele_off, ((size_t)x.V + 1) * 4, bi);
            UP(x.o_aid, b.allele_id, (size_t)x.sumA * 2, bi);
            UP(x.o_aflag, b.allele_flags, (size_t)x.sumA, bi);
            UP(x.o_akoff, b.allele_kmer_off, (size_t)x.sumA * 2, bi);
            UP(x.o_akmask, b.allele_kmer_mask, (size_t)x.sumA * 4, bi);
            UP(x.o_pa, b.path_allele, (size_t)x.V * x.H * 2, bi);
            UP(x.o_goff, x.goff.data(), ((size_t)x.V + 1) * 8, bi);
            if (x.wide_bytes) UP(x.o_widx, x.widx.data(), (size_t)x.V * 4, bi);
            if (x.aux_bytes) UP(x.o_auxidx, x.auxidx.data(), (size_t)x.V * 4, bi);
            UP(x.o_list_m4, x.list_m4.data(), x.list_m4.size() * 4, bi);
            UP(x.o_list_w, x.list_w.data(), x.list_w.size() * 4, bi);
            UP(x.o_list_b, x.list_b.data(), x.list_b.size() * 4, bi);
            UP(x.o_list_big, x.list_big.data(), x.list_big.size() * 4, bi);
        }
        cur_late = false;
        UP(job->o_tab_m, job->tab_m.data(), job->tab_m.size() * sizeof(double), bi);
        UP(job->o_tab_e, job->tab_e.data(), job->tab_e.size() * sizeof(int32_t), bi);
        UP(job->o_tab_p, job->tab_p.data(), job->tab_p.size(), bi);
    }
    if (job->cohort) {
        std::vector<std::vector<uint16_t>> cov(job->chains.size());
        const int rc = sample_upload(job, specs, job->cur_samples, s, &cov, &bs, err, errlen);
        if (rc != PG_OK) return rc;
        for (size_t c = 0; c < job->chains.size(); ++c) job->chains[c].coverage.swap(cov[c]);
    } else {
        const size_t rebase = (size_t)(job->cur_samples - (A + job->sample_lo));
        for (size_t c = 0; c < job->chains.size(); ++c) {
            ChainHost& ch = job->chains[c];
            const IndexHost& x = job->index[ch.index];
            if (x.V == 0) continue;
            cur_late = pipe && late[c];
            UP(ch.o_cov + rebase, specs[c].coverage, (size_t)x.V * 2, bs);
            UP(ch.o_kcnt + rebase, specs[c].kmer_count, (size_t)x.sumK * 2, bs);
            ch.coverage.assign(specs[c].coverage, specs[c].coverage + x.V);
        }
    }
#undef UP
    auto shares_of = [](const std::vector<Copy>& list, unsigned nt) {
        std::vector<std::vector<Copy>> share(nt);
        std::vector<size_t> load(nt, 0), order(list.size());
        for (size_t i = 0; i < order.size(); ++i) order[i] = i;
        std::sort(order.begin(), order.end(), [&](size_t x, size_t y) { return list[x].bytes > list[y].bytes; });
        for (size_t i : order) {
            unsigned best = 0;
            for (unsigned t = 1; t < nt; ++t) if (load[t] < load[best]) best = t;
            share[best].push_back(list[i]); load[best] += list[i].bytes;
        }
        return share;
    };
    const int device = job->device;
    auto copy_worker = [device](std::vector<Copy> mine, int* rc) {
        hipStream_t st = nullptr;
        hipError_t e = hipSetDevice(device);
        if (e == hipSuccess) e = hipStreamCreateWithFlags(&st, hipStreamNonBlocking);
        for (const Copy& c : mine) { if (e != hipSuccess) break; e = hipMemcpyAsync(c.dst, c.src, c.bytes, hipMemcpyDefault, st); }
        if (e == hipSuccess) e = hipStreamSynchronize(st);
        if (st) hipStreamDestroy(st);
        *rc = (int)e;
    };
    {
        size_t total = 0;
        for (const Copy& c : copies) total += c.bytes;
        for (const Copy& c : late_copies) total += c.bytes;
        const unsigned nt = (total >= ((size_t)64 << 20) && copies.size() + late_copies.size() >= 8) ? 4u : 1u;
        if (nt > 1) {
            std::vector<std::vector<Copy>> share = shares_of(copies, nt);
            std::vector<int> rcs(nt, (int)hipSuccess);
            std::vector<std::thread> th;
            for (unsigned t = 1; t < nt; ++t) th.emplace_back(copy_worker, share[t], &rcs[t]);
            copy_worker(share[0], &rcs[0]);
            for (auto& t : th) t.join();
            for (unsigned t = 0; t < nt; ++t)
                if (rcs[t] != (int)hipSuccess) { set_err(err, errlen, "input upload: %s", hipGetErrorString((hipError_t)rcs[t])); return PG_ERR_DEVICE; }
        } else {
            for (const Copy& c : copies) HIP_TRY(hipMemcpyAsync(c.dst, c.src, c.bytes, hipMemcpyDefault, s));
        }
        if (pipe) {
            hipStream_t st2 = job->stream2;
            auto staged_worker = [device, st2](std::vector<Copy> mine, int* rc) {
                hipStream_t st = st2;
                hipEvent_t ev[2] = {nullptr, nullptr};
                unsigned char* buf[2] = {g_pinned.get(), g_pinned.get()};
                hipError_t e = hipSetDevice(device);
                for (int k = 0; k < 2 && e == hipSuccess; ++k) e = hipEventCreateWithFlags(&ev[k], hipEventDisableTiming);
                if (e == hipSuccess && (!buf[0] || !buf[1])) e = hipErrorOutOfMemory;
                size_t piece = 0;
                for (const Copy& c : mine) {
                    if (e != hipSuccess) break;
                    hipPointerAttribute_t at;
                    const bool on_device = hipPointerGetAttributes(&at, c.src) == hipSuccess && at.type == hipMemoryTypeDevice;
                    if (!on_device) (void)hipGetLastError();
                    if (on_device) { e = hipMemcpyAsync(c.dst, c.src, c.bytes, hipMemcpyDeviceToDevice, st); continue; }
                    for (size_t off = 0; off < c.bytes && e == hipSuccess; off += PinnedPool::kBytes, ++piece) {
                        const size_t nby = std::min(PinnedPool::kBytes, c.bytes - off);
                        const int k = (int)(piece & 1u);
                        if (piece >= 2) e = hipEventSynchronize(ev[k]);
                        if (e != hipSuccess) break;
                        memcpy(buf[k], (const unsigned char*)c.src + off, nby);
                        e = hipMemcpyAsync((unsigned char*)c.dst + off, buf[k], nby, hipMemcpyHostToDevice, st);
                        if (e == hipSuccess) e = hipEventRecord(ev[k], st);
                    }
                }
                for (int k = 0; k < 2; ++k) if (ev[k] && piece > (size_t)k) { const hipError_t e2 = hipEventSynchronize(ev[k]); if (e == hipSuccess) e = e2; }
                for (int k = 0; k < 2; ++k) { if (ev[k]) hipEventDestroy(ev[k]); g_pinned.put(buf[k]); }
                *rc = (int)e;
            };
            const unsigned ntb = late_copies.size() >= 8 ? 4u : 1u;
            std::vector<std::vector<Copy>> share = shares_of(late_copies, ntb);
            job->late_rc.assign(ntb, (int)hipSuccess);
            job->late_threads.clear();
            for (unsigned t = 0; t < ntb; ++t) job->late_threads.emplace_back(staged_worker, share[t], &job->late_rc[t]);
            job->late_pending = true;
            late_guard.armed = true;
        }
    }
    HIP_TRY(hipStreamSynchronize(s));
    if (with_index) {
        HIP_TRY(hipEventRecord(job->ev_ix[0], s));
        HIP_TRY(hipMemsetAsync(job->ix_base, 0, job->ix_bytes, s));
        if (job->srec_bytes) HIP_TRY(hipMemsetAsync(job->srec_base, 0, job->srec_bytes, s));
        const uint32_t max_big = max_big_list(job);
        if (pipe) pgk_launch_index(job->d_reps_g, job->nA, job->max_v, max_big, 0, s);
        else pgk_launch_index(job->d_reps, (uint32_t)job->index.size(), job->max_v, max_big, job->any_split ? 1 : 0, s);
        HIP_TRY(hipGetLastError());
        HIP_TRY(hipEventRecord(job->ev_ix[1], s));
        HIP_TRY(hipStreamSynchronize(s));
        float ims = 0.f;
        HIP_TRY(hipEventElapsedTime(&ims, job->ev_ix[0], job->ev_ix[1]));
        job->index_ms = ims;
    }
    job->up_bytes[0] = bi; job->up_bytes[1] = bs;
    job->host_s[1] = now_s() - t0;
    late_guard.armed = false;
    return PG_OK;
}

struct KernelChoice {
    bool general = false, generic = false, nolean2 = false, notri = false, nocls4 = false, prepwave = false, fullcols = false, nosmall2 = false, nosplit = false;
    bool persist = false, noleanx2 = false, nowidef = false, nosparse = false, nosparse2 = false, nopieces = false;
    int leanx = -1, small = -1;
    std::string unknown;
};
KernelChoice kernel_choice() {
    KernelChoice k;
    const char* e = getenv("PG_KERNELS");
    if (!e) return k;
    std::string tok;
    auto take = [&]() {
        if (tok == "general") k.general = true; else if (tok == "generic") k.generic = true;
        else if (tok == "leanx") k.leanx = 1; else if (tok == "noleanx") k.leanx = 0;
        else if (tok == "small") k.small = 1; else if (tok == "nosmall") k.small = 0;
        else if (tok == "nolean2") k.nolean2 = true; else if (tok == "notri") k.notri = true;
        else if (tok == "nocls4") k.nocls4 = true; else if (tok == "prepwave") k.prepwave = true;
        else if (tok == "fullcols") k.fullcols = true; else if (tok == "nosmall2") k.nosmall2 = true;
        else if (tok == "nosplit") k.nosplit = true;
        else if (tok == "noleanx2") k.noleanx2 = true;
        else if (tok == "nowidef") k.nowidef = true;
        else if (tok == "nosparse") k.nosparse = true;
        else if (tok == "nosparse2") k.nosparse2 = true;
        else if (tok == "nopieces") k.nopieces = true;
        else if (tok == "persist") k.persist = true; else if (tok == "nopersist") k.persist = false;
        else if (!tok.empty()) k.unknown = tok;
        tok.clear();
    };
    for (const char* c = e; *c; ++c) { if (*c == ',' || *c == ' ') take(); else tok.push_back(*c); }
    take();
    return k;
}

template <class F>
void parallel_contigs(uint32_t n, const pg_contig_batch* batches, F&& f) {
    uint64_t total = 0;
    for (uint32_t i = 0; i < n; ++i) total += batches[i].n_variants;
    unsigned nt = std::thread::hardware_concurrency();
    nt = nt ? (nt > 16 ? 16 : nt) : 4;
    if (nt > n) nt = n;
    if (n < 2 || total < 200000 || nt < 2) { for (uint32_t i = 0; i < n; ++i) f(i); return; }
    std::atomic<uint32_t> next{0};
    std::vector<std::thread> th;
    auto work = [&]() { for (uint32_t i = next.fetch_add(1); i < n; i = next.fetch_add(1)) f(i); };
    for (unsigned t = 1; t < nt; ++t) th.emplace_back(work);
    work();
    for (auto& t : th) t.join();
}

struct BuildArgs {
    uint32_t n_index;
    const pg_contig_batch* batches;
    const std::vector<ChainSpec>& specs;
    const pg_hmm_params& params;
    KernelChoice kc;
    bool cohort, cache_arena;
};

struct JobOwner {
    pg_job* job;
    ~JobOwner() { if (job) pg_job_destroy(job); }
    pg_job* release() { pg_job* j = job; job = nullptr; return j; }
};

int hip_fail(char* err, size_t errlen, const char* what, hipError_t e) {
    set_err(err, errlen, "%s: %s", what, hipGetErrorString(e));
    return PG_ERR_DEVICE;
}

int check_inputs(uint32_t n_index, const pg_contig_batch* batches, const std::vector<ChainSpec>& specs, const pg_table* table,
                 const pg_hmm_params* params, bool cohort, char* err, size_t errlen) {
    if (!batches || !table || !params || n_index == 0 || specs.empty()) { set_err(err, errlen, "null argument"); return PG_ERR_INVALID; }
    if (params->run_phasing) {
        for (const ChainSpec& sp : specs)
            if (batches[sp.index].n_paths > 64u) {
                set_err(err, errlen, "run_phasing: %u selected paths, the device Viterbi takes at most 64", batches[sp.index].n_paths);
                return PG_ERR_UNSUPPORTED;
            }
    }
    {
        std::vector<int> rcs(n_index, PG_OK);
        std::vector<std::string> msgs(n_index);
        parallel_contigs(n_index, batches, [&](uint32_t i) {
            char e[256] = {0};
            rcs[i] = check_batch(&batches[i], !cohort, e, sizeof(e));
            if (rcs[i] != PG_OK) msgs[i] = e;
        });
        for (uint32_t i = 0; i < n_index; ++i)
            if (rcs[i] != PG_OK) { set_err(err, errlen, "%s", msgs[i].c_str()); return rcs[i]; }
    }
    for (const ChainSpec& sp : specs) {
        const pg_contig_batch& b = batches[sp.index];
        if (b.n_variants > 0 && (!sp.coverage || (b.kmer_off[b.n_variants] > 0 && !sp.kmer_count))) {
            set_err(err, errlen, "a chain has null kmer_count / coverage arrays");
            return PG_ERR_INVALID;
        }
    }
    return PG_OK;
}

int select_device(int device, char* err, size_t errlen) {
    int ndev = 0;
    if (hipGetDeviceCount(&ndev) != hipSuccess || ndev == 0) { set_err(err, errlen, "no HIP device available (no CPU fallback)"); return PG_ERR_DEVICE; }
    if (device < 0 || device >= ndev) { set_err(err, errlen, "bad device %d", device); return PG_ERR_INVALID; }
    if (hipSetDevice(device) != hipSuccess) { set_err(err, errlen, "hipSetDevice failed"); return PG_ERR_DEVICE; }
    return PG_OK;
}
// ... 177 lines not shown

enum SweepKernel : uint8_t {
    SW_NONE, SW_HP16, SW_HP32, SW_HP64, SW_HP128, SW_GENERIC, SW_GENERIC64, SW_LEAN, SW_LEAN_TRI, SW_LEAN2, SW_LEANX128, SW_LEANX64,
    SW_TRI1, SW_LEANX_TRI, SW_LEANX_TRIW, SW_LEANX2, SW_SMALL16, SW_SMALL16X, SW_COUNT
};
struct SweepRow { uint32_t bits; const char* name; bool phased; };
const SweepRow kSweep[SW_COUNT] = {
    {0u, "", false},
    {PG_SWEEP_HP16, "k_sweep<16,4>", true}, {PG_SWEEP_HP32, "k_sweep<32,8>", true},
    {PG_SWEEP_HP64, "k_sweep<64,16>", true}, {PG_SWEEP_HP128, "k_sweep<128,32>", true},
    {PG_SWEEP_GENERIC, "k_sweep_generic", true},
    {PG_SWEEP_GENERIC64 | PG_SWEEP_GENERIC , "k_sweep_generic", true},
    {PG_SWEEP_LEAN, "k_sweep_lean", true}, {PG_SWEEP_LEAN | PG_SWEEP_TRI, "k_sweep_lean_tri", true}, {PG_SWEEP_LEAN2, "k_sweep_lean2", false},
    {PG_SWEEP_LEANX128, "k_sweep_leanx", true}, {PG_SWEEP_LEANX64, "k_sweep_leanx", true},
    {PG_SWEEP_TRI1 | PG_SWEEP_TRI, "k_sweep_tri1", false}, {PG_SWEEP_LEANX_TRI | PG_SWEEP_TRI, "k_sweep_leanx_tri", false},
    {PG_SWEEP_LEANX_TRIW | PG_SWEEP_TRI, "k_sweep_leanx_triw", false}, {PG_SWEEP_LEANX2, "k_sweep_leanx2", false},
    {0u, "k_sweep_small16", true}, {0u, "k_sweep_small16x", true}
};
enum BinsKernel : uint8_t { BN_NONE, BN_FULL, BN_LEAN2, BN_THIN, BN_X, BN_WIDE, BN_S, BN_WIDE_S, BN_Q, BN_COUNT };
struct BinsRow { uint32_t bit; const char* name; };
const BinsRow kBins[BN_COUNT] = {{0u, ""}, {PG_BINS_FULL, "k_bins"}, {PG_BINS_LEAN2, "k_bins_lean2"}, {PG_BINS_THIN, "k_bins_thin"}, {PG_BINS_X, "k_bins_x"},
                                 {PG_BINS_WIDE, "k_bins_wide"}, {PG_BINS_S, "k_bins_s"}, {PG_BINS_WIDE_S, "k_bins_wide_s"}, {PG_BINS_Q, "k_bins_q"}};
enum PrepKernels : uint8_t { PREP_S_BI, PREP_S_LISTS, PREP_BI, PREP_BI_LISTS, PREP_W, PREP_COUNT };
const char* const kPrepName[PREP_COUNT] = {
    "index pass once (k_index_scan, k_compact, k_index_cols); per run k_prep_s_bi",
    "index pass once (k_index_scan, k_compact, k_index_cols); per run k_prep_s_bi + k_prep_s_m4 + k_prep_s_w",
    "index pass once (k_index_scan, k_compact); per run k_prep_bi + k_records",
    "index pass once (k_index_scan, k_compact); per run k_prep_bi + k_prep_m4 + k_prep + k_records",
    "index pass once (k_index_scan, k_compact); per run k_prep + k_records"
};
enum PostKernels : uint8_t { POST_NONE, POST_CHUNKS, POST_LOOP };

struct ChainKernels {
    PrepKernels prep = PREP_W;
    SweepKernel phase1 = SW_NONE;
    SweepKernel phase2 = SW_NONE;
    SweepKernel general = SW_NONE;
    PostKernels post = POST_NONE;
    BinsKernel bins = BN_NONE;
    BinsKernel bins_one = BN_NONE;
    BinsKernel bins_wide = BN_NONE;
    uint32_t lean = 0, leanx = 0, leanx2 = 0, tri = 0, cls4 = 0, small = 0, smallx = 0, widef = 0, T = 0, sparse = 0, sparse2 = 0;
};

std::vector<ChainKernels> choose_chain_kernels(pg_job* job, const BuildArgs& a) {
    const KernelChoice& kc = a.kc;
    const bool fused = !job->chunked;
    std::vector<ChainKernels> kernels(a.specs.size());
    job->hp_mask = 0; job->bins_which = 0; job->vit_bits = 0;
    for (size_t c = 0; c < kernels.size(); ++c) {
        const IndexHost& x = job->index[a.specs[c].index];
        ChainKernels& k = kernels[c];
        const bool tri_multi = !x.lean && !x.leanx && x.HP == 64 && x.H == 64 && (!x.wide_bytes || x.widef) && x.pair_n > 2 && !kc.generic && !kc.general;
        const bool tri = (x.lean || tri_multi) && fused && !kc.notri;
        k.lean = x.lean ? 1u : 0u; k.cls4 = x.cls4 ? 1u : 0u; k.widef = x.widef ? 1u : 0u; k.T = part_entries(x);
        k.small = x.small ? ((fused && x.cls4 && !kc.nosmall2) ? 2u : 1u) : 0u;
        k.smallx = x.smallx ? ((fused && !kc.nosmall2) ? 2u : 1u) : 0u;
        k.tri = tri ? ((kc.nolean2 || !x.lean) ? 1u : 2u) : 0u;
        if (k.tri == 1u && !x.lean && x.HP == 64u && !kc.noleanx2 && !a.params.run_phasing && !x.widef) { k.leanx2 = 1u; k.T = 64u; }
        k.leanx = (k.tri && !x.lean && kc.leanx != 0) ? 2u : (x.leanx ? 1u : 0u);
        k.sparse = (job->sparse && k.lean == 1u && k.tri == 0u) ? 1u : 0u;
        k.sparse2 = (job->sparse2 && k.sparse) ? 1u : 0u;
        k.prep = x.split ? (x.all_sb ? PREP_S_BI : PREP_S_LISTS) : x.prep_fast == 1u ? PREP_BI : x.prep_fast == 2u ? PREP_BI_LISTS : PREP_W;

        const SweepKernel own = x.HP >= 256 ? SW_GENERIC : (kc.generic && x.HP >= 64) ? SW_GENERIC64
                              : x.HP == 16 ? SW_HP16 : x.HP == 32 ? SW_HP32 : x.HP == 64 ? SW_HP64 : SW_HP128;
        const SweepKernel leanx_kernel = x.HP == 128 ? SW_LEANX128 : SW_LEANX64;
        const bool walked = own == SW_GENERIC || own == SW_GENERIC64 || (!x.split && !(job->chunked && (x.lean || x.small || x.smallx || x.leanx)));
        k.general = walked ? own : SW_NONE;
        k.phase1 = k.lean ? (k.tri ? SW_LEAN_TRI : SW_LEAN) : k.leanx == 2u ? (k.widef ? SW_LEANX_TRIW : SW_LEANX_TRI) : k.leanx ? leanx_kernel
                 : k.small ? SW_SMALL16 : k.smallx ? SW_SMALL16X : k.tri ? SW_TRI1 : own;
        if (fused) k.phase2 = k.leanx2 ? SW_LEANX2 : k.tri == 2u ? SW_LEAN2 : k.small == 2u ? SW_SMALL16 : k.smallx == 2u ? SW_SMALL16X : own;
        else k.phase2 = k.lean ? SW_LEAN : k.leanx ? leanx_kernel : k.small ? SW_SMALL16 : k.smallx ? SW_SMALL16X : own;
        k.post = fused ? POST_NONE : job->persist ? POST_LOOP : POST_CHUNKS;
        const BinsKernel own_bins = k.leanx2 ? BN_Q : (k.tri == 2u || k.cls4) ? BN_LEAN2 : (k.T <= 64u && x.HP <= 32u && fused) ? BN_THIN : BN_FULL;
        if (x.split) { k.bins = BN_S; k.bins_wide = (x.split == 2u && x.wide_bytes) ? BN_WIDE_S : BN_NONE; }
        else if (k.smallx == 2u) { k.bins = BN_X; k.bins_one = own_bins; k.bins_wide = x.wide_bytes ? BN_WIDE : BN_NONE; }
        else { k.bins = own_bins; k.bins_wide = (k.widef && x.n_wide_cand) ? BN_WIDE : BN_NONE; }

        job->hp_mask |= kSweep[k.phase1].bits | kSweep[k.phase2].bits | kSweep[k.general].bits;
        job->bins_which |= kBins[k.bins].bit | kBins[k.bins_one].bit | kBins[k.bins_wide].bit;
        if (a.params.run_phasing) job->vit_bits |= x.HP == 16 ? 1u : (x.HP == 32 ? 2u : 4u);
    }
    return kernels;
}

std::string sweep_name(SweepKernel k, int phase) {
    const SweepRow& n = kSweep[k];
    return n.phased ? std::string(n.name) + "<" + std::to_string(phase) + ">" : std::string(n.name);
}

std::string plan_text(const pg_job* job, const BuildArgs& a, const std::vector<ChainKernels>& kernels) {
    struct Group { std::string text; uint32_t count = 0; };
    std::vector<Group> groups;
    for (size_t c = 0; c < kernels.size(); ++c) {
        const IndexHost& x = job->index[a.specs[c].index];
        const ChainKernels& k = kernels[c];
        if (x.V == 0) continue;
        auto name = [&](SweepKernel s, int phase) { return sweep_name(a.kc.generic && s >= SW_HP16 && s <= SW_HP128 ? SW_GENERIC : s, phase); };
        std::string p2, bins;
        if (k.post == POST_LOOP) { p2 = name(k.phase2, 4) + " (one launch, all chunks) + k_post_loop"; bins = "(k_post_loop)"; }
        else if (k.post == POST_CHUNKS) { p2 = name(k.phase2, 3) + (k.sparse2 ? " chunks (sparse: every 64th column stored) + k_refill_lean (both halves) + " : k.sparse ? " chunks + k_refill_lean + " : " chunks + ") + "k_post"; bins = "(k_post)"; }
        else {
            p2 = name(k.phase2, 2);
            if (k.tri && k.phase2 == k.general) p2 += " (triangle ring)";
            if (k.widef) p2 += " (wide columns to their aux slots)";
            bins = kBins[k.bins].name;
            if (k.bins_wide) bins += std::string(" + ") + kBins[k.bins_wide].name;
        }
        char head[160];
        snprintf(head, sizeof(head), "%u path(s) (padded %u), %s%s%s columns: ", x.H, x.HP, x.pair_n > 2 ? "multiallelic" : "biallelic", x.wide_bytes ? " + wide" : "",
                 k.tri ? ", triangle" : "");
        const std::string text = std::string(head) + "prep = " + kPrepName[k.prep] + "; phase 1 = " + name(k.phase1, 1) + (k.sparse ? (k.sparse2 && job->n_pieces > 1u ? " (sparse: every 64th column stored, in " + std::to_string(job->n_pieces) + " pieces with k_refill_lean beside them)" : std::string(" (sparse: every 64th column stored)")) : std::string()) + "; phase 2 = " + p2 + "; bins = " + bins;
        bool found = false;
        for (auto& g : groups) if (g.text == text) { g.count += 1; found = true; break; }
        if (!found) groups.push_back({text, 1});
    }
    std::string out = std::string(job->chunked ? "chunked" : "fused") + " job, " + std::to_string(kernels.size()) + " chain(s)" + (a.params.run_phasing ? ", run_phasing (k_viterbi)" : "") + "\n";
    for (const auto& g : groups) out += "  " + std::to_string(g.count) + " x " + g.text + "\n";
    return out;
}

struct ChainOffsets { size_t sync, wcols, wlist, aux, frec, scratch, wide, vpair, xbuf, prof, fback, fscale, bscale, bsum, vrec, colrec, fwd, part, cprec,
                      vtq, vback, vbest, hap1, hap2, ckpt; };
struct ArenaLayout {
    size_t o_contigs, o_reps, o_contigs_g, o_reps_g, o_small, o_dump, o_handshake, o_err, o_lik, o_likexp, o_ncols, o_ixerr;
    size_t zero_lo, zero_hi, ix_lo, ix_hi, vrec_lo, vrec_hi, srec_lo, srec_hi;
    size_t bytes;
    std::vector<ChainOffsets> chain;
};

ArenaLayout layout_arena(pg_job* job, const BuildArgs& a, const std::vector<ChainKernels>& kernels) {
    const uint32_t n_chains = (uint32_t)a.specs.size(), n_index = a.n_index;
    const bool vit = a.params.run_phasing != 0;
    const bool geno = a.params.run_genotyping != 0;
    ArenaLayout L;
    L.chain.resize(n_chains);
    size_t off = 0;
    auto take = [&](size_t bytes, size_t al = 256) { off = align_up(off, al); size_t o = off; off += (bytes ? bytes : 8); return o; };
    L.o_contigs = take(sizeof(DevContig) * n_chains);
    L.o_reps = take(sizeof(DevContig) * n_index);
    L.o_contigs_g = take(sizeof(DevContig) * n_chains); L.o_reps_g = take(sizeof(DevContig) * n_index);
    L.o_small = take(sizeof(uint32_t) * n_chains);
    L.o_dump = take(64 * 8 * 16 + 8 * 16 * 16 * 16);
    L.o_handshake = take(64);
    L.zero_lo = align_up(off);
    L.o_err = take(sizeof(uint32_t) * n_chains);
    uint64_t lik_total = 0;
    for (uint32_t c = 0; c < n_chains; ++c) {
        ChainHost& ch = job->chains[c];
        const IndexHost& x = job->index[ch.index];
        ChainOffsets& p = L.chain[c];
        p.fback = take(x.V);
        p.prof = take(64 * sizeof(unsigned long long));
        p.wcols = take(4);
        p.sync = take(job->chunked ? PG_SYNC_WORDS * sizeof(uint32_t) : 0);
        p.vbest = take(vit ? 4 : 0);
        p.hap1 = take(vit ? (size_t)x.V * 2 : 0);
        p.hap2 = take(vit ? (size_t)x.V * 2 : 0);
        ch.lik_first = lik_total;
        lik_total += x.n_lik;
    }
    job->n_lik_total = lik_total;
    L.o_lik = take(lik_total * sizeof(double));
    L.o_likexp = take(lik_total * sizeof(int32_t));
    L.zero_hi = off;
    job->o_tab_m = take(job->tab_m.size() * sizeof(double));
    job->o_tab_e = take(job->tab_e.size() * sizeof(int32_t));
    job->o_tab_p = take(job->tab_p.size());
    L.ix_lo = align_up(off);
    L.o_ncols = take(sizeof(uint32_t) * n_index);
    L.o_ixerr = take(sizeof(uint32_t) * n_index);
    for (IndexHost& x : job->index) {
        x.o_kept = take(x.V); x.o_apres = take(x.sumA);
        x.o_colv = take((size_t)x.V * 4); x.o_colof = take((size_t)x.V * 4);
        x.o_ixpd = take(x.split ? (size_t)x.V * PG_IXPD_BYTES : 0);
        x.o_ixrec = take(x.split ? (size_t)x.V * PG_IXREC_BYTES : 0);
        x.o_ixbin = take(x.split ? (size_t)x.V * PG_IXBIN_BYTES : 0);
        x.o_ixwl = take(x.split == 2u && x.wide_bytes ? (size_t)x.n_wide_cand * 4 : 0);
        x.o_ixnw = take(4);
    }
    L.ix_hi = off > L.ix_lo ? off : L.ix_lo;
    for (IndexHost& x : job->index) {
        x.o_pos = take((size_t)x.V * 8);
        x.o_koff = take(((size_t)x.V + 1) * 4);
        x.o_aoff = take(((size_t)x.V + 1) * 4); x.o_aid = take((size_t)x.sumA * 2);
        x.o_aflag = take(x.sumA); x.o_akoff = take((size_t)x.sumA * 2); x.o_akmask = take((size_t)x.sumA * 4);
        x.o_pa = take((size_t)x.V * x.H * 2);
        x.o_goff = take(((size_t)x.V + 1) * 8);
        x.o_widx = take(x.wide_bytes ? (size_t)x.V * 4 : 0);
        x.o_auxidx = take(x.aux_bytes ? (size_t)x.V * 4 : 0);
        x.o_list_m4 = take(x.list_m4.size() * 4);
        x.o_list_w = take(x.list_w.size() * 4);
        x.o_list_b = take(x.list_b.size() * 4);
        x.o_list_big = take(x.list_big.size() * 4);
    }
    job->sample_lo = align_up(off);
    for (ChainHost& ch : job->chains) {
        const IndexHost& x = job->index[ch.index];
        ch.o_cov = take((size_t)x.V * 2); ch.o_kcnt = take((size_t)x.sumK * 2);
    }
// ... 3 lines not shown
    L.vrec_hi = off;
    L.srec_lo = align_up(off);
    for (uint32_t c = 0; c < n_chains; ++c) {
        const IndexHost& x = job->index[job->chains[c].index];
        if (x.split) L.chain[c].frec = take((size_t)x.V * (x.split == 1u ? PG_SREC1_BYTES : PG_SREC2_BYTES));
    }
    L.srec_hi = off > L.srec_lo ? off : L.srec_lo;
    for (uint32_t c = 0; c < n_chains; ++c) {
        const IndexHost& x = job->index[job->chains[c].index];
        const ChainKernels& k = kernels[c];
        ChainOffsets& p = L.chain[c];
        p.colrec = take(x.split ? 0 : (size_t)x.V * x.RB);
        p.cprec = take(x.split ? (size_t)x.V * PG_CPREC_BYTES : 0);
        p.fwd = take(geno ? (size_t)x.V * (k.tri ? 2304u : (size_t)x.HP * x.HP) * sizeof(double) : 0);
        const bool x2 = k.smallx == 2u;
        p.part = take(job->chunked || !geno ? 0 : (x2 ? (size_t)x.V * 32u + (size_t)x.part_slots * part_entries(x) * sizeof(double)
                                                      : (size_t)x.V * x.part_slots * part_entries(x) * sizeof(double)));
        p.aux = take((x2 || x.widef) && geno ? x.aux_bytes : 0);
        p.wlist = take((x2 || x.widef) && geno && x.wide_bytes && !x.split ? (size_t)x.n_wide_cand * 4 : 0);
        p.vtq = take(vit ? (size_t)x.V * 8 * sizeof(double) : 0);
        p.vback = take(vit ? (size_t)x.V * x.H * x.HP * sizeof(uint16_t) : 0);
        p.scratch = take(job->chunked ? (size_t)2 * PG_SCRATCH_BUFS * job->chunk_cols * x.HP * x.HP * sizeof(double) : 0);
        p.ckpt = take(k.sparse2 ? (size_t)2 * pg_sparse2_slots(x.V) * x.HP * x.HP * sizeof(double) : 0);
        p.wide = take(x.wide_bytes);
        p.vpair = take(x.split ? 0 : (size_t)x.V * pg_pair_bytes(x.pair_n));
        p.xbuf = take((x.HP >= 256 || (a.kc.generic && x.HP >= 64)) ? (size_t)2 * x.HP * x.HP * sizeof(double) : 0);
        if (!x.split) p.frec = take((x.lean || x.small) ? (size_t)x.V * 64 : (x.smallx ? (size_t)x.V * 192 : 0));
        p.fscale = take((size_t)x.V * sizeof(double));
        p.bscale = take((size_t)x.V * sizeof(double));
        p.bsum = take((size_t)x.V * sizeof(double));
    }
    L.bytes = align_up(off);
    return L;
}

hipError_t allocate_arena(pg_job* job, size_t bytes) {
    const double t0 = now_s();
    job->arena_bytes = bytes;
    if (job->cache_arena) g_pool.take(job->device, job->arena_bytes, &job->arena, &job->arena_bytes);
    hipError_t he = hipSuccess;
    if (!job->arena) {
        he = hipMalloc((void**)&job->arena, job->arena_bytes);
        if (he != hipSuccess) {
            (void)hipGetLastError();
            pg_hmm_release_cache();
            hipSetDevice(job->device);
            he = hipMalloc((void**)&job->arena, job->arena_bytes);
        }
        if (he != hipSuccess) { job->arena = nullptr; (void)hipGetLastError(); }
    }
    job->host_s[0] = now_s() - t0;
    return he;
}

int create_device_objects(pg_job* job, char* err, size_t errlen) {
    hipError_t he;
    if ((he = hipStreamCreate(&job->stream)) != hipSuccess) return hip_fail(err, errlen, "hipStreamCreate", he);
    for (auto& e : job->ev)
        if ((he = hipEventCreate(&e)) != hipSuccess) return hip_fail(err, errlen, "hipEventCreate", he);
    for (auto& e : job->ev_vit)
        if ((he = hipEventCreate(&e)) != hipSuccess) return hip_fail(err, errlen, "hipEventCreate", he);
    for (auto& e : job->ev_ix)
        if ((he = hipEventCreate(&e)) != hipSuccess) return hip_fail(err, errlen, "hipEventCreate", he);
    job->events = true;
    if (!job->chunked) return PG_OK;
    if ((he = hipStreamCreateWithFlags(&job->stream2, hipStreamNonBlocking)) != hipSuccess) return hip_fail(err, errlen, "hipStreamCreate", he);
    for (int q = 0; q < (int)PG_SCRATCH_BUFS; ++q) {
        if ((he = hipEventCreateWithFlags(&job->ev_sweep[q], hipEventDisableTiming)) != hipSuccess) return hip_fail(err, errlen, "hipEventCreate", he);
        if ((he = hipEventCreateWithFlags(&job->ev_post[q], hipEventDisableTiming)) != hipSuccess) return hip_fail(err, errlen, "hipEventCreate", he);
    }
    job->events2 = true;
    if (job->sparse2) {
        job->ev_chunk.reserve(job->n_chunks);
        for (uint32_t q = 0; q < job->n_chunks; ++q) {
            hipEvent_t e;
            if ((he = hipEventCreateWithFlags(&e, hipEventDisableTiming)) != hipSuccess) return hip_fail(err, errlen, "hipEventCreate", he);
            job->ev_chunk.push_back(e);
        }
        if (job->n_pieces > 1u) for (uint32_t g = 0; g < job->n_pieces; ++g) {
            hipEvent_t e;
            if ((he = hipEventCreateWithFlags(&e, hipEventDisableTiming)) != hipSuccess) return hip_fail(err, errlen, "hipEventCreate", he);
            job->ev_piece.push_back(e);
        }
    }
    return PG_OK;
}

void bind_arena(pg_job* job, const ArenaLayout& L) {
    unsigned char* A = job->arena;
    job->d_contigs = (DevContig*)(A + L.o_contigs);
    job->d_reps = (DevContig*)(A + L.o_reps);
    job->d_contigs_g = (DevContig*)(A + L.o_contigs_g); job->d_reps_g = (DevContig*)(A + L.o_reps_g);
    job->d_small = (uint32_t*)(A + L.o_small);
    job->d_dump = (double*)(A + L.o_dump);
    job->d_handshake = (uint32_t*)(A + L.o_handshake);
    job->d_ixerr = (uint32_t*)(A + L.o_ixerr);
    job->ix_base = A + L.ix_lo; job->ix_bytes = L.ix_hi - L.ix_lo;
    job->srec_base = A + L.srec_lo; job->srec_bytes = L.srec_hi - L.srec_lo;
    job->d_ncols = (uint32_t*)(A + L.o_ncols);
    job->d_err = (uint32_t*)(A + L.o_err);
    job->d_lik = (double*)(A + L.o_lik);
    job->d_likexp = (int32_t*)(A + L.o_likexp);
    job->zero_base = A + L.zero_lo;
    job->zero_bytes = L.zero_hi - L.zero_lo;
    job->tab.mant = (const double*)(A + job->o_tab_m);
    job->tab.expo = (const int32_t*)(A + job->o_tab_e);
    job->tab.packed = A + job->o_tab_p;
    job->cur_samples = A + job->sample_lo;
}

std::vector<DevContig> fill_descriptors(pg_job* job, const BuildArgs& a, const std::vector<ChainKernels>& kernels, const ArenaLayout& L) {
    unsigned char* A = job->arena;
    const pg_hmm_params& params = a.params;
    std::vector<DevContig> hd(job->chains.size());
    const long double dist_scale = 0.000004L * ((long double)params.recombrate) * params.effective_N;
    for (size_t c = 0; c < hd.size(); ++c) {
        ChainHost& ch = job->chains[c];
        const IndexHost& x = job->index[ch.index];
        const ChainOffsets& p = L.chain[c];
        const ChainKernels& k = kernels[c];
        DevContig& d = hd[c];
        memset(&d, 0, sizeof(d));
        d.V = x.V; d.H = x.H; d.HP = x.HP; d.RB = x.RB; d.T = k.T; d.part_slots = x.part_slots; d.pair_n = x.pair_n;
        d.dist_scale = (double)dist_scale; d.uniform = params.uniform ? 1 : 0;
        d.debug = 8u;
        d.pos = (const uint64_t*)(A + x.o_pos); d.cov = (const uint16_t*)(A + ch.o_cov);
        d.kmer_off = (const uint32_t*)(A + x.o_koff); d.kmer_count = (const uint16_t*)(A + ch.o_kcnt);
        d.allele_off = (const uint32_t*)(A + x.o_aoff); d.allele_id = (const uint16_t*)(A + x.o_aid);
        d.allele_flags = (const uint8_t*)(A + x.o_aflag); d.allele_koff = (const uint16_t*)(A + x.o_akoff);
        d.allele_kmask = (const uint32_t*)(A + x.o_akmask); d.path_allele = (const uint16_t*)(A + x.o_pa);
        d.geno_off = (const uint64_t*)(A + x.o_goff);
        d.vrec = A + p.vrec; d.kept = A + x.o_kept; d.allele_present = A + x.o_apres;
        d.n_cols = job->d_ncols + ch.index; d.col_variant = (uint32_t*)(A + x.o_colv); d.colrec = A + p.colrec;
        d.col_of = (const uint32_t*)(A + x.o_colof); d.ix_err = job->d_ixerr + ch.index;
        d.ix_big = (const uint32_t*)(A + x.o_list_big); d.n_ix_big = (uint32_t)x.list_big.size();
        d.split = x.split;
        if (x.split) {
            d.ix_pd = A + x.o_ixpd; d.ix_rec = A + x.o_ixrec; d.ix_bin = A + x.o_ixbin; d.cprec = A + p.cprec;
        }
        d.fwd = (double*)(A + p.fwd); d.part = (double*)(A + p.part); d.fwd_fallback = A + p.fback; d.prof = (unsigned long long*)(A + p.prof);
        d.fscale = (double*)(A + p.fscale); d.bscale = (double*)(A + p.bscale); d.bsum = (double*)(A + p.bsum); d.err = job->d_err + c;
        d.lik = job->d_lik + ch.lik_first; d.lik_exp = job->d_likexp + ch.lik_first;
        d.scratch = (double*)(A + p.scratch); d.chunk_cols = job->chunk_cols; d.sync = (uint32_t*)(A + p.sync);
        d.wide = A + p.wide; d.wide_idx = x.wide_bytes ? (const uint32_t*)(A + x.o_widx) : nullptr;
        d.vpair = A + p.vpair; d.xbuf = (double*)(A + p.xbuf);
        d.frec = (double*)(A + p.frec);
        d.lean = k.lean; d.small = k.small; d.smallx = k.smallx; d.leanx = k.leanx; d.leanx2 = k.leanx2; d.cls4 = k.cls4; d.widef = k.widef; d.tri = k.tri; d.sparse = k.sparse;
        d.sparse2 = k.sparse2; d.ckpt = (double*)(A + p.ckpt); d.ckpt_slots = pg_sparse2_slots(x.V);
        d.col_stride = d.tri ? 2304u : x.HP * x.HP;
        d.aux = A + p.aux; d.aux_idx = ((d.smallx == 2u || x.widef) && x.aux_bytes) ? (const uint32_t*)(A + x.o_auxidx) : nullptr;
        if ((d.smallx == 2u || x.widef) && x.wide_bytes && x.n_wide_cand) {
            if (x.split) { d.wcols = (uint32_t*)(A + x.o_ixwl); d.n_wcols = (uint32_t*)(A + x.o_ixnw); }
            else { d.wcols = (uint32_t*)(A + p.wlist); d.n_wcols = (uint32_t*)(A + p.wcols); }
            job->max_wide = std::max(job->max_wide, x.n_wide_cand);
        }
        d.live = (!job->chunked && x.HP == 32u && !a.kc.fullcols) ? std::min<uint32_t>(x.HP, (x.H + 3u) & ~3u) : x.HP;
        d.prep_fast = x.prep_fast;
        if (k.prep == PREP_S_LISTS || k.prep == PREP_BI_LISTS) {
            d.prep_m4 = (const uint32_t*)(A + x.o_list_m4); d.n_prep_m4 = (uint32_t)x.list_m4.size();
            d.prep_w = (const uint32_t*)(A + x.o_list_w); d.n_prep_w = (uint32_t)x.list_w.size();
            d.prep_b = (const uint32_t*)(A + x.o_list_b); d.n_prep_b = (uint32_t)x.list_b.size();
        }
        if (x.split) {
            job->max_sb = std::max(job->max_sb, k.prep == PREP_S_BI ? x.V : d.n_prep_b);
            job->max_sm4 = std::max(job->max_sm4, d.n_prep_m4);
            job->max_sw = std::max(job->max_sw, d.n_prep_w);
// ... 445 lines not shown
}

extern "C" int pg_job_device_results(pg_job* job, uint32_t ci, void** d_lik, uint64_t* n_lik, void** d_lik_exp, uint64_t* n_variants) {
    if (!job || ci >= job->chains.size()) return PG_ERR_INVALID;
    const ChainHost& c = job->chains[ci];
    const IndexHost& x = job->index[c.index];
    if (d_lik) *d_lik = c.d.lik;
    if (n_lik) *n_lik = x.n_lik;
    if (d_lik_exp) *d_lik_exp = c.d.lik_exp;
    if (n_variants) *n_variants = x.V;
    return PG_OK;
}

extern "C" int pg_job_packed_results(pg_job* job, void** d_lik, void** d_lik_exp, uint64_t* n_lik_total) {
    if (!job) return PG_ERR_INVALID;
    if (d_lik) *d_lik = job->d_lik;
    if (d_lik_exp) *d_lik_exp = job->d_likexp;
    if (n_lik_total) *n_lik_total = job->n_lik_total;
    return PG_OK;
}

extern "C" uint32_t pg_job_n_chains(const pg_job* job) { return job ? (uint32_t)job->chains.size() : 0; }

extern "C" int pg_job_host_seconds(const pg_job* job, double out4[4]) {
    if (!job || !out4) return PG_ERR_INVALID;
    for (int i = 0; i < 4; ++i) out4[i] = job->host_s[i];
    return PG_OK;
}
extern "C" int pg_job_upload_bytes(const pg_job* job, uint64_t out2[2]) {
    if (!job || !out2) return PG_ERR_INVALID;
    out2[0] = job->up_bytes[0]; out2[1] = job->up_bytes[1];
    return PG_OK;
}

extern "C" int pg_job_profile_counters(pg_job* job, uint32_t ci, uint64_t out64[64]) {
    if (!job || !out64 || ci >= job->chains.size()) return PG_ERR_INVALID;
    if (hipSetDevice(job->device) != hipSuccess) return PG_ERR_DEVICE;
    if (hipMemcpy(out64, job->chains[ci].d.prof, 64 * sizeof(uint64_t), hipMemcpyDeviceToHost) != hipSuccess) return PG_ERR_DEVICE;
    return PG_OK;
}

extern "C" int pg_job_kernel_ms(const pg_job* job, double ms[PG_N_KERNEL_CLASSES]) {
    if (!job || !ms) return PG_ERR_INVALID;
    for (int i = 0; i < PG_N_KERNEL_CLASSES; ++i) ms[i] = job->ms[i];
    return PG_OK;
}
extern "C" const char* pg_job_kernel_name(int cls) { return (cls >= 0 && cls < PG_N_KERNEL_CLASSES) ? kKernelNames[cls] : ""; }
extern "C" uint64_t pg_job_device_bytes(const pg_job* job) { return job ? job->arena_bytes : 0; }
extern "C" int pg_job_sweep_mode(const pg_job* job, uint32_t* chunk_cols) {
    if (!job) return PG_ERR_INVALID;
    if (chunk_cols) *chunk_cols = job->chunk_cols;
    return job->chunked ? 1 : 0;
}

extern "C" double pg_job_viterbi_ms(const pg_job* job) { return job ? job->vit_ms : 0.0; }

extern "C" double pg_job_index_ms(const pg_job* job) { return job ? job->index_ms : 0.0; }
extern "C" size_t pg_job_plan(const pg_job* job, char* out, size_t len) {
    if (!job) return 0;
    std::string t = job->plan_text;
    if (job->persist) {
        char line[160];
        snprintf(line, sizeof(line), "  persistent phase 2: %u run(s), %u more fell back to a launch per chunk\n", job->persist_runs, job->persist_fallbacks);
        t += line;
    }
    if (out && len) { const size_t n = t.size() < len - 1 ? t.size() : len - 1; memcpy(out, t.data(), n); out[n] = 0; }
    return t.size() + 1;
}
extern "C" int pg_sparse_segment(uint32_t n_columns, uint32_t chunk_cols, uint32_t chunk, uint32_t role, uint32_t j, uint32_t out[3]) {
    if (role > 1u || chunk_cols == 0u || chunk_cols % PG_LEAN_SPARSE != 0u || j >= chunk_cols / PG_LEAN_SPARSE) return -1;
    const unsigned long long m = (unsigned long long)chunk * (chunk_cols / PG_LEAN_SPARSE) + j + 1u;
    if (m > pg_sparse_segments(n_columns, role)) return 0;
    const uint32_t ck = pg_sparse_checkpoint(n_columns, role, (uint32_t)m);
    if (out) { out[0] = ck; out[1] = role == 0u ? ck + 1u : ck - (PG_LEAN_SPARSE - 1u); out[2] = role == 0u ? ck + (PG_LEAN_SPARSE - 1u) : ck - 1u; }
    return 1;
}
extern "C" int pg_sparse_piece_range(uint32_t n_columns, uint32_t chunk_cols, uint32_t piece_chunks, uint32_t piece, uint32_t role, uint32_t out[2]) {
    if (role > 1u || chunk_cols == 0u || chunk_cols % PG_LEAN_SPARSE != 0u || piece_chunks == 0u || (unsigned long long)piece_chunks * chunk_cols > 0xFFFFFFFFull) return -1;
    uint32_t r[2];
    if (!pg_sparse_piece(n_columns, role, piece_chunks * chunk_cols, piece, r)) return 0;
    if (out) { out[0] = r[0]; out[1] = r[1]; }
    return 1;
}
extern "C" int pg_sparse_chunk_segment(uint32_t n_columns, uint32_t chunk_cols, uint32_t chunk, uint32_t role, uint32_t j, uint32_t out[3]) {
    if (role > 1u || chunk_cols == 0u || chunk_cols % PG_LEAN_SPARSE != 0u || j >= chunk_cols / PG_LEAN_SPARSE) return -1;
    uint32_t seg[3];
    if (!pg_sparse2_segment(n_columns, role, (unsigned long long)chunk * (chunk_cols / PG_LEAN_SPARSE) + j, seg)) return 0;
    if (out) { out[0] = seg[0]; out[1] = seg[1]; out[2] = seg[2]; }
    return 1;
}
extern "C" int pg_sparse_chunk_stored_by_chain(uint32_t n_columns, uint32_t role, uint32_t column) {
    return role <= 1u && column < n_columns && pg_sparse2_stored(n_columns, role, column) ? 1 : 0;
}
extern "C" int pg_sparse_stored_by_chain(uint32_t n_columns, uint32_t role, uint32_t column) {
    return role <= 1u && column < n_columns && pg_sparse_stored(n_columns, role, column) ? 1 : 0;
}
extern "C" uint32_t pg_job_triangle_chains(const pg_job* job) {
    if (!job) return 0;
    uint32_t n = 0;
    for (const auto& ch : job->chains) n += ch.d.tri ? 1u : 0u;
    return n;
}

namespace {

int genotype_single(const pg_contig_batch* batch, const pg_table* table, const pg_hmm_params* params, int device,
                    pg_contig_result* out, char* err, size_t errlen) {
    std::vector<ChainSpec> specs(1);
    specs[0] = {0, batch->kmer_count, batch->coverage};
    pg_job* job = nullptr;
    int rc = job_build(device, 1, batch, specs, 1, false, table, params, true, &job, err, errlen);
    if (rc != PG_OK) return rc;
    rc = pg_job_run(job, nullptr, err, errlen);
    if (rc == PG_OK) rc = pg_job_fetch(job, 0, out, err, errlen);
    pg_job_destroy(job);
    return rc;
}

struct CoRequest {
    const pg_contig_batch* batch; pg_contig_result* out; char* err; size_t errlen;
    int rc = PG_OK; bool done = false;
};
struct CoBatch {
    int device; const pg_table* table; pg_hmm_params params;
    std::vector<CoRequest*> reqs;
    std::chrono::steady_clock::time_point last_arrival;
};
struct Coalescer {
    std::mutex mu;
    std::condition_variable cv;
    std::vector<std::shared_ptr<CoBatch>> open;
    int callers_inside = 0;
    int announced[PG_MAX_DEVICES_HOST] = {0};
    int inflight[PG_MAX_DEVICES_HOST] = {0};
    std::chrono::steady_clock::time_point last_concurrency = std::chrono::steady_clock::time_point::min();
    uint64_t stat_batches = 0, stat_requests = 0, stat_largest = 0;
} g_co;

long env_long(const char* name, long dflt) { const char* e = getenv(name); return e ? strtol(e, nullptr, 0) : dflt; }

bool same_params(const pg_hmm_params& a, const pg_hmm_params& b) {
    return a.effective_N == b.effective_N && a.recombrate == b.recombrate && (a.uniform != 0) == (b.uniform != 0) &&
           (a.run_genotyping != 0) == (b.run_genotyping != 0) && (a.run_phasing != 0) == (b.run_phasing != 0);
}

void run_merged(CoBatch& b) {
    const size_t n = b.reqs.size();
    pg_hmm_params prm = b.params;
    prm.reserved = 0;
    if (n > 1) {
        std::vector<pg_contig_batch> bs(n);
        std::vector<ChainSpec> specs(n);
        for (size_t i = 0; i < n; ++i) { bs[i] = *b.reqs[i]->batch; specs[i] = {(uint32_t)i, bs[i].kmer_count, bs[i].coverage}; }
        char err[512] = {0};
        pg_job* job = nullptr;
        int rc = job_build(b.device, (uint32_t)n, bs.data(), specs, 1, false, b.table, &prm, true, &job, err, sizeof(err));
        if (rc == PG_OK) rc = pg_job_run(job, nullptr, err, sizeof(err));
        if (rc == PG_OK) {
            std::vector<pg_contig_result> outs(n);
            for (size_t i = 0; i < n; ++i) outs[i] = *b.reqs[i]->out;
            rc = pg_job_fetch_all(job, outs.data(), err, sizeof(err));
            for (size_t i = 0; i < n; ++i) b.reqs[i]->out->n_columns = outs[i].n_columns;
        }
        if (job) pg_job_destroy(job);
        if (rc == PG_OK) { for (CoRequest* r : b.reqs) r->rc = PG_OK; return; }
    }
// ... 150 lines not shown
```

pangenie_amd/csrc/pg_shim_run.cpp:

```cpp
#include <hip/hip_runtime_api.h>

#include <math.h>

#include <algorithm>
#include <vector>

#include "pg_job.h"

using namespace pgj;

#define STEP(call)                        \
    do {                                  \
        const int rc_ = (call);           \
        if (rc_ != PG_OK) return rc_;     \
    } while (0)

namespace pgj __attribute__((visibility("hidden"))) {
bool streams_concurrent(pg_job* job, hipStream_t s) {
    if (job->persist_checked_any && job->persist_checked == s) return true;
    for (int attempt = 0; attempt < 6; ++attempt) {
        uint32_t w[4] = {0, 0, 0, 0};
        if (hipMemcpyAsync(job->d_handshake, w, sizeof(w), hipMemcpyHostToDevice, s) != hipSuccess || hipStreamSynchronize(s) != hipSuccess) break;
        pgk_launch_stream_handshake(job->d_handshake, s, job->stream2);
        if (hipGetLastError() != hipSuccess || hipStreamSynchronize(s) != hipSuccess || hipStreamSynchronize(job->stream2) != hipSuccess) break;
        if (hipMemcpy(w, job->d_handshake, sizeof(w), hipMemcpyDeviceToHost) != hipSuccess) break;
        if (w[2] == 1u) { job->persist_checked = s; job->persist_checked_any = true; return true; }
        hipStream_t fresh = nullptr;
        if (hipStreamCreateWithFlags(&fresh, hipStreamNonBlocking) != hipSuccess) break;
        (void)hipStreamDestroy(job->stream2);
        job->stream2 = fresh;
    }
    (void)hipGetLastError();
    return false;
}
}

namespace {

struct RunPlan {
    bool genotype = false;
    bool index_b_due = false;
    bool persist_now = false;
    bool pieces_now = false;
};

int join_late_checked(pg_job* job, char* err, size_t errlen) {
    join_late_threads(job);
    for (int rcb : job->late_rc)
        if (rcb != (int)hipSuccess) { set_err(err, errlen, "input upload: %s", hipGetErrorString((hipError_t)rcb)); return PG_ERR_DEVICE; }
    return PG_OK;
}

int settle_late_for_callers_stream(pg_job* job, hipStream_t s, RunPlan* plan, char* err, size_t errlen) {
    plan->index_b_due = job->late_pending && s != job->stream;
    if (!plan->index_b_due) return PG_OK;
    STEP(join_late_checked(job, err, errlen));
    HIP_TRY(hipEventRecord(job->ev_late[1], job->stream2));
    HIP_TRY(hipStreamWaitEvent(s, job->ev_late[1], 0));
    return PG_OK;
}

int first_run_pipelined(pg_job* job, hipStream_t s, char* err, size_t errlen) {
    const uint32_t n = (uint32_t)job->chains.size(), nA = job->nA, nB = n - nA;
    HIP_TRY(hipEventRecord(job->ev_late[0], s));
    pgk_launch_prep(job->d_contigs_g, nA, job->max_v, job->max_prep_w, job->max_prep_m4, job->tab, s);
    HIP_TRY(hipGetLastError());
    HIP_TRY(hipEventRecord(job->ev[1], s));
    HIP_TRY(hipEventRecord(job->ev[2], s));
    pgk_launch_records(job->d_contigs_g, nA, job->max_v, s);
    HIP_TRY(hipGetLastError());
    HIP_TRY(hipEventRecord(job->ev[3], s));
    pgk_launch_sweep(job->d_contigs_g, nA, job->hp_mask, 1, s);
    HIP_TRY(hipGetLastError());
    STEP(join_late_checked(job, err, errlen));
    hipStream_t sb = job->stream2;
    HIP_TRY(hipStreamWaitEvent(sb, job->ev_late[0], 0));
    pgk_launch_index(job->d_reps_g + nA, nB, job->max_v, max_big_list(job), 0, sb);
    pgk_launch_prep(job->d_contigs_g + nA, nB, job->max_v, job->max_prep_w, job->max_prep_m4, job->tab, sb);
    pgk_launch_records(job->d_contigs_g + nA, nB, job->max_v, sb);
    pgk_launch_sweep(job->d_contigs_g + nA, nB, job->hp_mask, 1, sb);
    HIP_TRY(hipGetLastError());
    HIP_TRY(hipEventRecord(job->ev_late[1], sb));
    HIP_TRY(hipStreamWaitEvent(s, job->ev_late[1], 0));
    HIP_TRY(hipEventRecord(job->ev[4], s));
    return PG_OK;
}

int prepare(pg_job* job, hipStream_t s, bool index_b_due, char* err, size_t errlen) {
    const uint32_t n = (uint32_t)job->chains.size();
    if (index_b_due) {
        pgk_launch_index(job->d_reps_g + job->nA, n - job->nA, job->max_v, max_big_list(job), 0, s);
        HIP_TRY(hipGetLastError());
    }
    if (job->any_legacy_prep) pgk_launch_prep(job->d_contigs, n, job->max_v, job->max_prep_w, job->max_prep_m4, job->tab, s);
    if (job->any_split) pgk_launch_prep_split(job->d_contigs, n, job->max_sb, job->max_sm4, job->max_sw, job->tab, s);
    HIP_TRY(hipGetLastError());
    HIP_TRY(hipEventRecord(job->ev[1], s));
    HIP_TRY(hipEventRecord(job->ev[2], s));
    if (job->any_legacy_prep) pgk_launch_records(job->d_contigs, n, job->max_v, s);
    HIP_TRY(hipGetLastError());
    HIP_TRY(hipEventRecord(job->ev[3], s));
    return PG_OK;
}

int phase1_in_pieces(pg_job* job, hipStream_t s, char* err, size_t errlen) {
    const uint32_t n = (uint32_t)job->chains.size(), G = job->piece_chunks;
    if (job->hp_mask & ~PG_SWEEP_LEAN) pgk_launch_sweep(job->d_contigs, n, job->hp_mask & ~PG_SWEEP_LEAN, 1, s);
    for (uint32_t g = job->n_pieces; g-- > 0u;) {
        pgk_launch_sweep_piece(job->d_contigs, n, G, g, s);
        HIP_TRY(hipGetLastError());
        HIP_TRY(hipEventRecord(job->ev_piece[g], s));
        if (g == 0u) break;
        HIP_TRY(hipStreamWaitEvent(job->stream2, job->ev_piece[g], 0));
        for (uint32_t i = std::min((g + 1u) * G, job->n_chunks); i-- > g * G;) pgk_launch_refill(job->d_contigs, n, job->chunk_cols, i, 0, job->piece_refill_blocks, job->stream2);
        HIP_TRY(hipGetLastError());
    }
    return PG_OK;
}

int phase1(pg_job* job, hipStream_t s, RunPlan* plan, char* err, size_t errlen) {
    const uint32_t n = (uint32_t)job->chains.size();
    plan->pieces_now = job->n_pieces > 1u && s == job->stream;
    if (plan->pieces_now) STEP(phase1_in_pieces(job, s, err, errlen));
    else pgk_launch_sweep(job->d_contigs, n, job->hp_mask, 1, s);
    pgk_launch_sweep_small(job->d_contigs, job->d_small, job->n_small, 1, 0, job->d_dump, s);
    pgk_launch_sweep_smallx(job->d_contigs, job->d_smallx, job->n_smallx, 1, 0, job->d_dump, s);
    HIP_TRY(hipGetLastError());
    HIP_TRY(hipEventRecord(job->ev[4], s));
    return PG_OK;
}

int phase2_fused(pg_job* job, hipStream_t s, char* err, size_t errlen) {
    const uint32_t n = (uint32_t)job->chains.size();
    pgk_launch_sweep(job->d_contigs, n, job->hp_mask, 2, s);
    if (job->small_phase2) pgk_launch_sweep_small(job->d_contigs, job->d_small, job->n_small, 2, 0, job->d_dump, s);
    if (job->smallx_phase2) pgk_launch_sweep_smallx(job->d_contigs, job->d_smallx, job->n_smallx, 2, 0, job->d_dump, s);
    HIP_TRY(hipGetLastError());
    HIP_TRY(hipEventRecord(job->ev[5], s));
    pgk_launch_bins(job->d_contigs, n, job->max_v, job->bins_which, job->max_wide, s);
    HIP_TRY(hipGetLastError());
    HIP_TRY(hipEventRecord(job->ev[6], s));
    return PG_OK;
}

int end_chunked_phase2(pg_job* job, hipStream_t s, char* err, size_t errlen) {
    HIP_TRY(hipEventRecord(job->ev[5], s));
    HIP_TRY(hipEventRecord(job->ev[6], s));
    return PG_OK;
}

int phase2_persistent(pg_job* job, hipStream_t s, char* err, size_t errlen) {
    const uint32_t n = (uint32_t)job->chains.size();
    hipStream_t s2 = job->stream2;
    HIP_TRY(hipStreamWaitEvent(s2, job->ev[4], 0));
    pgk_launch_phase2_persistent(job->d_contigs, n, job->post_blocks, s, s2);
    HIP_TRY(hipGetLastError());
    HIP_TRY(hipEventRecord(job->ev_post[0], s2));
    HIP_TRY(hipStreamWaitEvent(s, job->ev_post[0], 0));
    return end_chunked_phase2(job, s, err, errlen);
}

int phase2_sparse(pg_job* job, hipStream_t s, const RunPlan& plan, char* err, size_t errlen) {
    const uint32_t n = (uint32_t)job->chains.size();
    hipStream_t s2 = job->stream2;
    if (job->sparse) HIP_TRY(hipStreamWaitEvent(s2, job->ev[4], 0));
    for (uint32_t i = 0; i < job->n_chunks; ++i) {
        pgk_launch_sweep_chunk(job->d_contigs, n, job->hp_mask, i, s);
        HIP_TRY(hipGetLastError());
        HIP_TRY(hipEventRecord(job->ev_chunk[i], s));
        if (!plan.pieces_now || i < job->piece_chunks) pgk_launch_refill(job->d_contigs, n, job->chunk_cols, i, 0, 0u, s2);
        HIP_TRY(hipStreamWaitEvent(s2, job->ev_chunk[i], 0));
        pgk_launch_refill(job->d_contigs, n, job->chunk_cols, i, 1, 0u, s2);
        pgk_launch_post(job->d_contigs, n, job->chunk_cols, i, s2);
        HIP_TRY(hipGetLastError());
        if (i + 1u == job->n_chunks) {
            HIP_TRY(hipEventRecord(job->ev_post[0], s2));
            HIP_TRY(hipStreamWaitEvent(s, job->ev_post[0], 0));
        }
    }
    return end_chunked_phase2(job, s, err, errlen);
}

int phase2_chunks(pg_job* job, hipStream_t s, char* err, size_t errlen) {
    const uint32_t n = (uint32_t)job->chains.size();
    hipStream_t s2 = job->stream2;
    if (job->sparse) HIP_TRY(hipStreamWaitEvent(s2, job->ev[4], 0));
    for (uint32_t i = 0; i < job->n_chunks; ++i) {
        const int b = (int)PG_SCR_BUF(i);
        if (i >= PG_SCRATCH_BUFS) HIP_TRY(hipStreamWaitEvent(s, job->ev_post[b], 0));
        pgk_launch_sweep_chunk(job->d_contigs, n, job->hp_mask, i, s);
        pgk_launch_sweep_small(job->d_contigs, job->d_small, job->n_small, 3, i, job->d_dump, s);
        pgk_launch_sweep_smallx(job->d_contigs, job->d_smallx, job->n_smallx, 3, i, job->d_dump, s);
        HIP_TRY(hipGetLastError());
        HIP_TRY(hipEventRecord(job->ev_sweep[b], s));
        if (job->sparse) pgk_launch_refill(job->d_contigs, n, job->chunk_cols, i, 0, 0u, s2);
        HIP_TRY(hipStreamWaitEvent(s2, job->ev_sweep[b], 0));
        pgk_launch_post(job->d_contigs, n, job->chunk_cols, i, s2);
        HIP_TRY(hipGetLastError());
        HIP_TRY(hipEventRecord(job->ev_post[b], s2));
    }
    for (uint32_t q = 0; q < PG_SCRATCH_BUFS && q < job->n_chunks; ++q) HIP_TRY(hipStreamWaitEvent(s, job->ev_post[q], 0));
    return end_chunked_phase2(job, s, err, errlen);
}

int records_only(pg_job* job, hipStream_t s, char* err, size_t errlen) {
    pgk_launch_prep(job->d_contigs, (uint32_t)job->chains.size(), job->max_v, job->max_prep_w, job->max_prep_m4, job->tab, s);
// ... 34 lines not shown
                    tq[(size_t)k * 8 + 2 * q + 1] = (double)(t[q] - (long double)hi);
                }
            }
        }
        if (!tq.empty()) HIP_TRY(hipMemcpyAsync(ch.d.vit_tq, tq.data(), tq.size() * sizeof(double), hipMemcpyHostToDevice, s));
    }
    HIP_TRY(hipStreamSynchronize(s));
    return PG_OK;
}

int phase_viterbi(pg_job* job, hipStream_t s, char* err, size_t errlen) {
    if (!job->vit_tq_ready) {
        HIP_TRY(hipStreamSynchronize(s));
        if (job->stream2) HIP_TRY(hipStreamSynchronize(job->stream2));
        STEP(viterbi_transitions(job, s, err, errlen));
        job->vit_tq_ready = true;
    }
    HIP_TRY(hipEventRecord(job->ev_vit[0], s));
    pgk_launch_viterbi(job->d_contigs, (uint32_t)job->chains.size(), job->max_v, job->vit_bits, s);
    HIP_TRY(hipGetLastError());
    HIP_TRY(hipEventRecord(job->ev_vit[1], s));
    return PG_OK;
}

int read_timings(pg_job* job, const RunPlan& plan, char* err, size_t errlen) {
    if (plan.genotype) {
        for (int i = 0; i < PG_N_KERNEL_CLASSES; ++i) {
            float ms = 0.f;
            HIP_TRY(hipEventElapsedTime(&ms, job->ev[i], job->ev[i + 1]));
            job->ms[i] = ms;
        }
    }
    if (job->max_v > 0 && job->params.run_phasing) {
        float ms = 0.f;
        HIP_TRY(hipEventElapsedTime(&ms, job->ev_vit[0], job->ev_vit[1]));
        job->vit_ms = ms;
    }
    return PG_OK;
}

struct DevErr { uint32_t bit; int rc; const char* fmt; int arg; };
const DevErr kDevErrs[] = {
    {PG_DEVERR_ALLELE_NOT_FOUND, PG_ERR_INVALID, "chain %u: a path_allele value is not in the variant's allele list", 0},
    {PG_DEVERR_TOO_MANY_ALLELES, PG_ERR_UNSUPPORTED, "chain %u: a variant has more than %d alleles (device limit)", PG_MAX_ALLELES_PER_VARIANT},
    {PG_DEVERR_SYNC_TIMEOUT, PG_ERR_DEVICE, "chain %u: the persistent phase-2 kernels lost each other (a chunk flag did not arrive within 10 s); without PG_KERNELS=persist phase 2 takes a launch per chunk", 0},
    {PG_DEVERR_WIDE_FUSED, PG_ERR_UNSUPPORTED, "chain %u: its only column carries more than %d alleles on the selected paths, which a fused job cannot genotype (PG_SWEEP_MODE=chunked)", PG_AMAX},
    {PG_DEVERR_TOO_MANY_LOCAL, PG_ERR_UNSUPPORTED, "chain %u: a column has more than %d distinct alleles on the selected paths (device limit)", PG_WIDE_MAX},
};

int read_errors(pg_job* job, double t_run, char* err, size_t errlen) {
    const uint32_t n = (uint32_t)job->chains.size();
    std::vector<uint32_t> ncols(n), errs(n);
    {
        const size_t ni = job->index.size();
        std::vector<uint32_t> nc_ix(ni), err_ix(ni);
        HIP_TRY(hipMemcpy(nc_ix.data(), job->d_ncols, sizeof(uint32_t) * ni, hipMemcpyDeviceToHost));
        HIP_TRY(hipMemcpy(err_ix.data(), job->d_ixerr, sizeof(uint32_t) * ni, hipMemcpyDeviceToHost));
        HIP_TRY(hipMemcpy(errs.data(), job->d_err, sizeof(uint32_t) * n, hipMemcpyDeviceToHost));
        for (uint32_t i = 0; i < n; ++i) { ncols[i] = nc_ix[job->chains[i].index]; errs[i] |= err_ix[job->chains[i].index]; }
    }
    job->ran = true;
    job->host_s[2] = now_s() - t_run;
    for (uint32_t i = 0; i < n; ++i) {
        job->chains[i].n_cols_host = ncols[i];
        for (const DevErr& e : kDevErrs)
            if (errs[i] & e.bit) { set_err(err, errlen, e.fmt, i, e.arg); return e.rc; }
    }
    return PG_OK;
}

}

extern "C" int pg_job_run(pg_job* job, void* stream_, char* err, size_t errlen) {
    if (!job) { set_err(err, errlen, "null job"); return PG_ERR_INVALID; }
    const double t_run = now_s();
    HIP_TRY(hipSetDevice(job->device));
    hipStream_t s = stream_ ? (hipStream_t)stream_ : job->stream;
    job->host_s[3] = 0.0;
    RunPlan plan;
    plan.genotype = job->max_v > 0 && job->params.run_genotyping;
    STEP(settle_late_for_callers_stream(job, s, &plan, err, errlen));
    plan.persist_now = job->persist && plan.genotype && streams_concurrent(job, s);
    if (job->persist && plan.genotype) (plan.persist_now ? job->persist_runs : job->persist_fallbacks) += 1;
    HIP_TRY(hipMemsetAsync(job->zero_base, 0, job->zero_bytes, s));
    if (plan.genotype) {
        HIP_TRY(hipEventRecord(job->ev[0], s));
        if (job->late_pending) {
            STEP(first_run_pipelined(job, s, err, errlen));
        } else {
            STEP(prepare(job, s, plan.index_b_due, err, errlen));
            STEP(phase1(job, s, &plan, err, errlen));
        }
        if (!job->chunked) STEP(phase2_fused(job, s, err, errlen));
        else if (plan.persist_now) STEP(phase2_persistent(job, s, err, errlen));
        else if (job->sparse2) STEP(phase2_sparse(job, s, plan, err, errlen));
        else STEP(phase2_chunks(job, s, err, errlen));
    } else if (job->max_v > 0) {
        STEP(records_only(job, s, err, errlen));
    }
    if (job->max_v > 0 && job->params.run_phasing) STEP(phase_viterbi(job, s, err, errlen));
    HIP_TRY(hipStreamSynchronize(s));
    if (job->stream2) HIP_TRY(hipStreamSynchronize(job->stream2));
    STEP(read_timings(job, plan, err, errlen));
    return read_errors(job, t_run, err, errlen);
}
```

Measured before the change: 23.92 million.

## Split prep into end and middle parts, overlapping middle prep with first sweep pieces

Splits the per-variant prep and record building into two parts. The chain ends, which the first sweep pieces need, run ahead on the main stream. The middle band runs on a second stream concurrently with the first E sweep pieces, and the main stream waits on an event before it reaches the pieces that need it. The intent is to hide prep latency behind the piece-wise forward sweep instead of serialising it. In exchange it adds synchronous device-to-host reads of the part extents on the first run, extra kernel launches, and new cross-stream dependencies.

```diff
diff --git a/include/pangenie_hmm.h b/include/pangenie_hmm.h
--- a/include/pangenie_hmm.h
+++ b/include/pangenie_hmm.h
@@ -97,6 +97,9 @@
 int pg_sparse_chunk_segment(uint32_t n_columns, uint32_t chunk_cols, uint32_t chunk, uint32_t role, uint32_t j, uint32_t out[3]);
 int pg_sparse_chunk_stored_by_chain(uint32_t n_columns, uint32_t role, uint32_t column);
 int pg_sparse_piece_range(uint32_t n_columns, uint32_t chunk_cols, uint32_t piece_chunks, uint32_t piece, uint32_t role, uint32_t out[2]);
+int pg_prep_parts(uint32_t n_columns, uint32_t chunk_cols, uint32_t piece_chunks, uint32_t n_pieces, uint32_t early,
+                  const uint32_t* col_variant, uint32_t n_variants, uint32_t out_cols[2], uint32_t out_vars[2]);
+uint32_t pg_prep_part_member(uint32_t part, uint32_t lo, uint32_t hi, uint32_t n, uint32_t u);
 double pg_job_viterbi_ms(const pg_job* job);
 void pg_job_destroy(pg_job* job);
 
diff --git a/pangenie_amd/_lib.py b/pangenie_amd/_lib.py
--- a/pangenie_amd/_lib.py
+++ b/pangenie_amd/_lib.py
@@ -148,6 +148,10 @@
     lib.pg_sparse_chunk_stored_by_chain.restype = C.c_int
     lib.pg_sparse_piece_range.argtypes = [C.c_uint32, C.c_uint32, C.c_uint32, C.c_uint32, C.c_uint32, u32p]
     lib.pg_sparse_piece_range.restype = C.c_int
+    lib.pg_prep_parts.argtypes = [C.c_uint32, C.c_uint32, C.c_uint32, C.c_uint32, C.c_uint32, u32p, C.c_uint32, u32p, u32p]
+    lib.pg_prep_parts.restype = C.c_int
+    lib.pg_prep_part_member.argtypes = [C.c_uint32] * 5
+    lib.pg_prep_part_member.restype = C.c_uint32
     lib.pg_job_kernel_ms.argtypes = [C.c_void_p, f64p]
     lib.pg_job_kernel_ms.restype = C.c_int
     lib.pg_job_kernel_name.argtypes = [C.c_int]
@@ -296,6 +300,7 @@
     "pg_job_record_gl_ms", "pg_record_gl_from_bins", "pg_gl_from_values", "pg_gl_text",
     "pg_job_record_plan_strided", "pg_job_record_first", "pg_job_fetch_record_calls_packed", "pg_job_fetch_record_gl_packed",
     "pg_sparse_segment", "pg_sparse_stored_by_chain", "pg_sparse_chunk_segment", "pg_sparse_chunk_stored_by_chain", "pg_sparse_piece_range",
+    "pg_prep_parts", "pg_prep_part_member",
 ]
 
 
diff --git a/pangenie_amd/csrc/pg_device.h b/pangenie_amd/csrc/pg_device.h
--- a/pangenie_amd/csrc/pg_device.h
+++ b/pangenie_amd/csrc/pg_device.h
@@ -205,6 +205,26 @@
     else { out[0] = (uint32_t)(mid + d0); out[1] = (uint32_t)(mid + d1 - 1u); }
     return true;
 }
+#define PG_PREP_EARLY_PIECES_DEFAULT 2u
+PG_HD inline uint32_t pg_prep_band(uint32_t n_pieces, uint32_t E, uint32_t piece_cols) {
+    const unsigned long long W = (unsigned long long)(n_pieces - E) * piece_cols;
+    return W > 0xFFFFFFC0ull ? 0xFFFFFFC0u : (uint32_t)W;
+}
+PG_HD inline void pg_prep_middle(uint32_t C, uint32_t W, uint32_t out[2]) {
+    const uint32_t mid = C / 2u;
+    out[0] = mid - (mid < W ? mid : W);
+    out[1] = mid + (C - mid < W ? C - mid : W);
+}
+PG_HD inline void pg_prep_middle_variants(const uint32_t* col_variant, uint32_t C, uint32_t V, uint32_t W, uint32_t out[2]) {
+    uint32_t cr[2];
+    pg_prep_middle(C, W, cr);
+    out[0] = cr[0] == 0u ? 0u : col_variant[cr[0]];
+    out[1] = cr[1] >= C ? V : col_variant[cr[1]];
+}
+PG_HD inline uint32_t pg_prep_part_item(uint32_t part, uint32_t lo, uint32_t hi, uint32_t N, uint32_t u) {
+    if (part == 2u) return u < hi - lo ? lo + u : N;
+    return u < lo ? u : (u < N - (hi - lo) ? u + (hi - lo) : N);
+}
 
 PG_HD inline uint32_t pg_sparse2_slots(uint32_t V) { return (V / 2u + 1u) / PG_LEAN_SPARSE + 2u; }
 PG_HD inline bool pg_sparse2_segment(uint32_t C, uint32_t role, unsigned long long m, uint32_t out[3]) {
diff --git a/pangenie_amd/csrc/pg_job.h b/pangenie_amd/csrc/pg_job.h
--- a/pangenie_amd/csrc/pg_job.h
+++ b/pangenie_amd/csrc/pg_job.h
@@ -173,6 +173,11 @@
     uint32_t piece_chunks = 0, n_pieces = 1;
     uint32_t piece_refill_blocks = 0;
     std::vector<hipEvent_t> ev_piece;
+    bool prep_beside = false;
+    uint32_t prep_early = 0, prep_W = 0;
+    bool prep_parts_ready = false;
+    uint32_t prep_max_v[2] = {0, 0}, prep_max_c[2] = {0, 0};
+    hipEvent_t ev_prep2 = nullptr;
     bool pipeline = false, pipeline_capable = false, late_pending = false;
     uint32_t nA = 0;
     std::vector<uint32_t> grp_order;
diff --git a/pangenie_amd/csrc/pg_kernels.hip b/pangenie_amd/csrc/pg_kernels.hip
--- a/pangenie_amd/csrc/pg_kernels.hip
+++ b/pangenie_amd/csrc/pg_kernels.hip
@@ -586,13 +586,14 @@
 }
 DEVI int row_last_i32(int v) { return __builtin_amdgcn_update_dpp(v, v, 0x15F, 0xF, 0xF, true); }
 
-DEVI void prep_bi_unit(const DevContig& dc, const DevTable& tab, uint32_t unit) {
+template <bool PART = false>
+DEVI void prep_bi_unit(const DevContig& dc, const DevTable& tab, uint32_t unit, uint32_t part = 0u, uint32_t npart = 0u, uint32_t plo = 0u, uint32_t phi = 0u) {
     const uint32_t lane = threadIdx.x & 63u, grp = lane >> 4, l = lane & 15u;
-    const uint32_t nobj = dc.prep_b ? dc.n_prep_b : dc.V;
+    const uint32_t nobj = PART ? npart : (dc.prep_b ? dc.n_prep_b : dc.V);
     const uint32_t pos = unit * 16u + (threadIdx.x >> 6) * 4u + grp;
     if (unit * 16u + (threadIdx.x >> 6) * 4u >= nobj) return;
     bool live = pos < nobj;
-    const uint32_t v = dc.prep_b ? dc.prep_b[live ? pos : nobj - 1u] : pos;
+    const uint32_t v = PART ? pg_prep_part_item(part, plo, phi, dc.V, live ? pos : nobj - 1u) : (dc.prep_b ? dc.prep_b[live ? pos : nobj - 1u] : pos);
     const uint32_t vv = live ? v : dc.V - 1u;
     const uint32_t H = dc.H, HP = dc.HP;
     const uint32_t a0 = dc.allele_off[vv];
@@ -1030,12 +1031,13 @@
     return ((dc.tri == 2u || dc.small == 2u || dc.smallx == 2u) && C >= 2u) || (dc.lean && dc.tri == 0u && dc.chunk_cols > 0u);
 }
 
-DEVI void records_unit(const DevContig& dc, uint32_t unit) {
+template <bool PART = false>
+DEVI void records_unit(const DevContig& dc, uint32_t unit, uint32_t part = 0u, uint32_t plo = 0u, uint32_t phi = 0u) {
     const uint32_t wave = threadIdx.x >> 6, lane = threadIdx.x & 63;
     const uint32_t C = *dc.n_cols;
     if (dc.split) return;
     if (compact_records_only(dc, C) && !dc.smallx) {
-        const uint32_t c = unit * 256u + threadIdx.x;
+        const uint32_t c = PART ? pg_prep_part_item(part, plo, phi, C, unit * 256u + threadIdx.x) : unit * 256u + threadIdx.x;
         if (c >= C) return;
         const uint32_t v = dc.col_variant[c];
         const uint64_t* src = (const uint64_t*)(dc.vrec + (size_t)v * dc.RB);
@@ -1053,6 +1055,7 @@
         out[3] = f64x2{__longlong_as_double((long long)E[PG_ESTRIDE + 1]), __longlong_as_double((long long)src[PG_REC_BITS1 / 8])};
         return;
     }
+    if constexpr (PART) return;
     __shared__ double s_c[4][64][4];
     __shared__ uint32_t s_v[4][64];
     const uint32_t cbase = (unit * 4u + wave) * 64u;
@@ -6181,6 +6184,23 @@
                                from64 ? 64u : 256u);
     }
 }
+__global__ __launch_bounds__(256) void k_prep_bi_part(const DevContig* __restrict__ contigs, DevTable tab, uint32_t part, uint32_t W) {
+    const DevContig& dc = contigs[blockIdx.y];
+    if (dc.prep_fast != 1u || dc.split || dc.prep_b || dc.V == 0u) return;
+    uint32_t vr[2];
+    pg_prep_middle_variants(dc.col_variant, *dc.n_cols, dc.V, W, vr);
+    const uint32_t npart = part == 2u ? vr[1] - vr[0] : dc.V - (vr[1] - vr[0]);
+#pragma unroll 1
+    for (uint32_t r = 0; r < (uint32_t)PG_VREP; ++r) prep_bi_unit<true>(dc, tab, blockIdx.x * (uint32_t)PG_VREP + r, part, npart, vr[0], vr[1]);
+}
+__global__ __launch_bounds__(256) void k_records_part(const DevContig* __restrict__ contigs, uint32_t part, uint32_t W) {
+    const DevContig& dc = contigs[blockIdx.y];
+    if (dc.V == 0u) return;
+    uint32_t cr[2];
+    pg_prep_middle(*dc.n_cols, W, cr);
+    records_unit<true>(dc, blockIdx.x, part, cr[0], cr[1]);
+}
+
 extern "C" {
 
 void pgk_launch_prep(const DevContig* d_contigs, uint32_t n_contigs, uint32_t max_v, uint32_t max_w, uint32_t max_m4, DevTable tab, hipStream_t s) {
@@ -6212,6 +6232,12 @@
 void pgk_launch_records(const DevContig* d_contigs, uint32_t n_contigs, uint32_t max_v, hipStream_t s) {
     dim3 grid((max_v + 255) / 256, n_contigs);
     hipLaunchKernelGGL(k_records, grid, dim3(256), 0, s, d_contigs);
+}
+void pgk_launch_prep_part(const DevContig* d_contigs, uint32_t n_contigs, uint32_t part, uint32_t W, uint32_t max_pv, DevTable tab, hipStream_t s) {
+    if (max_pv) hipLaunchKernelGGL(k_prep_bi_part, dim3((uint32_t)(((unsigned long long)max_pv + 16 * PG_VREP - 1) / (16 * PG_VREP)), n_contigs), dim3(256), 0, s, d_contigs, tab, part, W);
+}
+void pgk_launch_records_part(const DevContig* d_contigs, uint32_t n_contigs, uint32_t part, uint32_t W, uint32_t max_pc, hipStream_t s) {
+    if (max_pc) hipLaunchKernelGGL(k_records_part, dim3((max_pc + 255u) / 256u, n_contigs), dim3(256), 0, s, d_contigs, part, W);
 }
 void pgk_launch_bins(const DevContig* d_contigs, uint32_t n_contigs, uint32_t max_v, uint32_t which, uint32_t max_wide, hipStream_t s) {
     const bool full = which & PG_BINS_FULL;
diff --git a/pangenie_amd/csrc/pg_launch.h b/pangenie_amd/csrc/pg_launch.h
--- a/pangenie_amd/csrc/pg_launch.h
+++ b/pangenie_amd/csrc/pg_launch.h
@@ -76,6 +76,8 @@
 void pgk_launch_index(const DevContig* d_reps, uint32_t n_index, uint32_t max_v, uint32_t max_big, int any_split, hipStream_t s);
 void pgk_launch_prep_split(const DevContig* d_contigs, uint32_t n_contigs, uint32_t max_b, uint32_t max_m4, uint32_t max_w, DevTable tab, hipStream_t s);
 void pgk_launch_records(const DevContig* d_contigs, uint32_t n_contigs, uint32_t max_v, hipStream_t s);
+void pgk_launch_prep_part(const DevContig* d_contigs, uint32_t n_contigs, uint32_t part, uint32_t W, uint32_t max_pv, DevTable tab, hipStream_t s);
+void pgk_launch_records_part(const DevContig* d_contigs, uint32_t n_contigs, uint32_t part, uint32_t W, uint32_t max_pc, hipStream_t s);
 void pgk_launch_bins(const DevContig* d_contigs, uint32_t n_contigs, uint32_t max_v, uint32_t which, uint32_t max_wide, hipStream_t s);
 void pgk_launch_sweep(const DevContig* d_contigs, uint32_t n_contigs, uint32_t hp_mask, int phase, hipStream_t s);
 void pgk_launch_sweep_piece(const DevContig* d_contigs, uint32_t n_contigs, uint32_t piece_chunks, uint32_t piece, hipStream_t s);
diff --git a/pangenie_amd/csrc/pg_shim.cpp b/pangenie_amd/csrc/pg_shim.cpp
--- a/pangenie_amd/csrc/pg_shim.cpp
+++ b/pangenie_amd/csrc/pg_shim.cpp
@@ -294,6 +294,7 @@
         for (int q = 0; q < (int)PG_SCRATCH_BUFS; ++q) { hipEventDestroy(job->ev_sweep[q]); hipEventDestroy(job->ev_post[q]); }
     for (hipEvent_t e : job->ev_chunk) hipEventDestroy(e);
     for (hipEvent_t e : job->ev_piece) hipEventDestroy(e);
+    if (job->ev_prep2) hipEventDestroy(job->ev_prep2);
     if (job->arena) {
         if (job->cache_arena) g_pool.put(job->device, job->arena, job->arena_bytes);
         else hipFree(job->arena);
@@ -397,6 +398,7 @@
     } while (0)
     if (with_index) {
         record_plans_changed(job);
+        job->prep_parts_ready = false;
         for (size_t i = 0; i < job->index.size(); ++i) {
             const pg_contig_batch& b = batches[i];
             IndexHost& x = job->index[i];
@@ -543,7 +545,7 @@
 
 struct KernelChoice {
     bool general = false, generic = false, nolean2 = false, notri = false, nocls4 = false, prepwave = false, fullcols = false, nosmall2 = false, nosplit = false;
-    bool persist = false, noleanx2 = false, nowidef = false, nosparse = false, nosparse2 = false, nopieces = false;
+    bool persist = false, noleanx2 = false, nowidef = false, nosparse = false, nosparse2 = false, nopieces = false, prepahead = false;
     int leanx = -1, small = -1;
     std::string unknown;
 };
@@ -565,6 +567,7 @@
         else if (tok == "nosparse") k.nosparse = true;
         else if (tok == "nosparse2") k.nosparse2 = true;
         else if (tok == "nopieces") k.nopieces = true;
+        else if (tok == "prepahead") k.prepahead = true;
         else if (tok == "persist") k.persist = true; else if (tok == "nopersist") k.persist = false;
         else if (!tok.empty()) k.unknown = tok;
         tok.clear();
@@ -908,6 +911,18 @@
         job->bins_which |= kBins[k.bins].bit | kBins[k.bins_one].bit | kBins[k.bins_wide].bit;
         if (a.params.run_phasing) job->vit_bits |= x.HP == 16 ? 1u : (x.HP == 32 ? 2u : 4u);
     }
+    job->prep_beside = false; job->prep_early = 0; job->prep_W = 0; job->prep_parts_ready = false;
+    if (job->n_pieces > 1u && !kc.prepahead) {
+        bool only_bi = true;
+        for (size_t c = 0; c < kernels.size(); ++c) if (job->index[a.specs[c].index].V && kernels[c].prep != PREP_BI) only_bi = false;
+        uint32_t E = PG_PREP_EARLY_PIECES_DEFAULT;
+        if (const char* e = getenv("PG_PREP_EARLY_PIECES")) { const long v = strtol(e, nullptr, 0); if (v >= 1 && v <= 0xFFFF) E = (uint32_t)v; }
+        if (only_bi && job->n_pieces >= E + 1u) {
+            job->prep_beside = true;
+            job->prep_early = E;
+            job->prep_W = pg_prep_band(job->n_pieces, E, job->piece_chunks * job->chunk_cols);
+        }
+    }
     return kernels;
 }
 
@@ -942,7 +957,11 @@
         for (auto& g : groups) if (g.text == text) { g.count += 1; found = true; break; }
         if (!found) groups.push_back({text, 1});
     }
-    std::string out = std::string(job->chunked ? "chunked" : "fused") + " job, " + std::to_string(kernels.size()) + " chain(s)" + (a.params.run_phasing ? ", run_phasing (k_viterbi)" : "") + "\n";
+    std::string out = std::string(job->chunked ? "chunked" : "fused") + " job, " + std::to_string(kernels.size()) + " chain(s)" + (a.params.run_phasing ? ", run_phasing (k_viterbi)" : "") +
+                      (job->max_v == 0 || !a.params.run_genotyping ? std::string()
+                       : job->prep_beside ? ", prep in parts: the ends of the chains ahead of the sweeps, their middle beside the first " + std::to_string(job->prep_early) + " of " +
+                                            std::to_string(job->n_pieces) + " pieces (k_prep_bi_part, k_records_part; on the job's own stream)"
+                                          : std::string(", prep ahead of the sweeps")) + "\n";
     for (const auto& g : groups) out += "  " + std::to_string(g.count) + " x " + g.text + "\n";
     return out;
 }
@@ -1112,6 +1131,7 @@
             if ((he = hipEventCreateWithFlags(&e, hipEventDisableTiming)) != hipSuccess) return hip_fail(err, errlen, "hipEventCreate", he);
             job->ev_piece.push_back(e);
         }
+        if (job->prep_beside && (he = hipEventCreateWithFlags(&job->ev_prep2, hipEventDisableTiming)) != hipSuccess) return hip_fail(err, errlen, "hipEventCreate", he);
     }
     return PG_OK;
 }
@@ -1723,6 +1743,23 @@
     if (out) { out[0] = r[0]; out[1] = r[1]; }
     return 1;
 }
+extern "C" int pg_prep_parts(uint32_t n_columns, uint32_t chunk_cols, uint32_t piece_chunks, uint32_t n_pieces, uint32_t early,
+                             const uint32_t* col_variant, uint32_t n_variants, uint32_t out_cols[2], uint32_t out_vars[2]) {
+    if (chunk_cols == 0u || chunk_cols % PG_LEAN_SPARSE != 0u || piece_chunks == 0u || (unsigned long long)piece_chunks * chunk_cols > 0xFFFFFFFFull) return -1;
+    if (early == 0u || n_pieces == 0u || n_columns > n_variants) return -1;
+    if (n_pieces < early + 1u) return 0;
+    const uint32_t W = pg_prep_band(n_pieces, early, piece_chunks * chunk_cols);
+    if (out_cols) pg_prep_middle(n_columns, W, out_cols);
+    if (out_vars) {
+        if (!col_variant && n_columns) return -1;
+        pg_prep_middle_variants(col_variant, n_columns, n_variants, W, out_vars);
+    }
+    return 1;
+}
+extern "C" uint32_t pg_prep_part_member(uint32_t part, uint32_t lo, uint32_t hi, uint32_t n, uint32_t u) {
+    if ((part != 1u && part != 2u) || lo > hi || hi > n) return n;
+    return pg_prep_part_item(part, lo, hi, n, u);
+}
 extern "C" int pg_sparse_chunk_segment(uint32_t n_columns, uint32_t chunk_cols, uint32_t chunk, uint32_t role, uint32_t j, uint32_t out[3]) {
     if (role > 1u || chunk_cols == 0u || chunk_cols % PG_LEAN_SPARSE != 0u || j >= chunk_cols / PG_LEAN_SPARSE) return -1;
     uint32_t seg[3];
diff --git a/pangenie_amd/csrc/pg_shim_run.cpp b/pangenie_amd/csrc/pg_shim_run.cpp
--- a/pangenie_amd/csrc/pg_shim_run.cpp
+++ b/pangenie_amd/csrc/pg_shim_run.cpp
@@ -42,6 +42,7 @@
     bool index_b_due = false;
     bool persist_now = false;
     bool pieces_now = false;
+    bool prep_beside_now = false;
 };
 
 int join_late_checked(pg_job* job, char* err, size_t errlen) {
@@ -103,10 +104,56 @@
     return PG_OK;
 }
 
-int phase1_in_pieces(pg_job* job, hipStream_t s, char* err, size_t errlen) {
+int prep_part_extents(pg_job* job, char* err, size_t errlen) {
+    if (job->prep_parts_ready) return PG_OK;
+    std::vector<char> done(job->index.size(), 0);
+    uint32_t mv[2] = {0, 0}, mc[2] = {0, 0};
+    for (const ChainHost& ch : job->chains) {
+        const IndexHost& x = job->index[ch.index];
+        if (x.V == 0 || done[ch.index]) continue;
+        done[ch.index] = 1;
+        uint32_t C = 0, cr[2], vr[2] = {0u, x.V};
+        HIP_TRY(hipMemcpy(&C, ch.d.n_cols, sizeof(uint32_t), hipMemcpyDeviceToHost));
+        if (C > x.V) { set_err(err, errlen, "index contig %u: bad column count", ch.index); return PG_ERR_DEVICE; }
+        pg_prep_middle(C, job->prep_W, cr);
+        if (cr[0] > 0u) HIP_TRY(hipMemcpy(&vr[0], ch.d.col_variant + cr[0], sizeof(uint32_t), hipMemcpyDeviceToHost));
+        if (cr[1] < C) HIP_TRY(hipMemcpy(&vr[1], ch.d.col_variant + cr[1], sizeof(uint32_t), hipMemcpyDeviceToHost));
+        if (vr[0] > vr[1] || vr[1] > x.V) { set_err(err, errlen, "index contig %u: bad column list", ch.index); return PG_ERR_DEVICE; }
+        mc[0] = std::max(mc[0], C - (cr[1] - cr[0])); mc[1] = std::max(mc[1], cr[1] - cr[0]);
+        mv[0] = std::max(mv[0], x.V - (vr[1] - vr[0])); mv[1] = std::max(mv[1], vr[1] - vr[0]);
+    }
+    for (int p = 0; p < 2; ++p) { job->prep_max_v[p] = mv[p]; job->prep_max_c[p] = mc[p]; }
+    job->prep_parts_ready = true;
+    return PG_OK;
+}
+
+int prepare_in_parts(pg_job* job, hipStream_t s, char* err, size_t errlen) {
+    const uint32_t n = (uint32_t)job->chains.size(), W = job->prep_W;
+    hipStream_t s2 = job->stream2;
+    pgk_launch_prep_part(job->d_contigs, n, 1u, W, job->prep_max_v[0], job->tab, s);
+    HIP_TRY(hipGetLastError());
+    HIP_TRY(hipEventRecord(job->ev[1], s));
+    HIP_TRY(hipEventRecord(job->ev[2], s));
+    pgk_launch_records_part(job->d_contigs, n, 1u, W, job->prep_max_c[0], s);
+    HIP_TRY(hipGetLastError());
+    HIP_TRY(hipEventRecord(job->ev[3], s));
+    HIP_TRY(hipStreamWaitEvent(s2, job->ev[3], 0));
+    pgk_launch_prep_part(job->d_contigs, n, 2u, W, job->prep_max_v[1], job->tab, s2);
+    pgk_launch_records_part(job->d_contigs, n, 2u, W, job->prep_max_c[1], s2);
+    HIP_TRY(hipGetLastError());
+    HIP_TRY(hipEventRecord(job->ev_prep2, s2));
+    return PG_OK;
+}
+
+int phase1_in_pieces(pg_job* job, hipStream_t s, bool beside, char* err, size_t errlen) {
     const uint32_t n = (uint32_t)job->chains.size(), G = job->piece_chunks;
-    if (job->hp_mask & ~PG_SWEEP_LEAN) pgk_launch_sweep(job->d_contigs, n, job->hp_mask & ~PG_SWEEP_LEAN, 1, s);
+    const uint32_t others = job->hp_mask & ~PG_SWEEP_LEAN;
+    if (others && !beside) pgk_launch_sweep(job->d_contigs, n, others, 1, s);
     for (uint32_t g = job->n_pieces; g-- > 0u;) {
+        if (beside && g + 1u + job->prep_early == job->n_pieces) {
+            HIP_TRY(hipStreamWaitEvent(s, job->ev_prep2, 0));
+            if (others) pgk_launch_sweep(job->d_contigs, n, others, 1, s);
+        }
         pgk_launch_sweep_piece(job->d_contigs, n, G, g, s);
         HIP_TRY(hipGetLastError());
         HIP_TRY(hipEventRecord(job->ev_piece[g], s));
@@ -121,7 +168,7 @@
 int phase1(pg_job* job, hipStream_t s, RunPlan* plan, char* err, size_t errlen) {
     const uint32_t n = (uint32_t)job->chains.size();
     plan->pieces_now = job->n_pieces > 1u && s == job->stream;
-    if (plan->pieces_now) STEP(phase1_in_pieces(job, s, err, errlen));
+    if (plan->pieces_now) STEP(phase1_in_pieces(job, s, plan->prep_beside_now, err, errlen));
     else pgk_launch_sweep(job->d_contigs, n, job->hp_mask, 1, s);
     pgk_launch_sweep_small(job->d_contigs, job->d_small, job->n_small, 1, 0, job->d_dump, s);
     pgk_launch_sweep_smallx(job->d_contigs, job->d_smallx, job->n_smallx, 1, 0, job->d_dump, s);
@@ -322,13 +369,16 @@
     STEP(settle_late_for_callers_stream(job, s, &plan, err, errlen));
     plan.persist_now = job->persist && plan.genotype && streams_concurrent(job, s);
     if (job->persist && plan.genotype) (plan.persist_now ? job->persist_runs : job->persist_fallbacks) += 1;
+    plan.prep_beside_now = plan.genotype && job->prep_beside && s == job->stream && !job->late_pending;
+    if (plan.prep_beside_now) STEP(prep_part_extents(job, err, errlen));
     HIP_TRY(hipMemsetAsync(job->zero_base, 0, job->zero_bytes, s));
     if (plan.genotype) {
         HIP_TRY(hipEventRecord(job->ev[0], s));
         if (job->late_pending) {
             STEP(first_run_pipelined(job, s, err, errlen));
         } else {
-            STEP(prepare(job, s, plan.index_b_due, err, errlen));
+            if (plan.prep_beside_now) STEP(prepare_in_parts(job, s, err, errlen));
+            else STEP(prepare(job, s, plan.index_b_due, err, errlen));
             STEP(phase1(job, s, &plan, err, errlen));
         }
         if (!job->chunked) STEP(phase2_fused(job, s, err, errlen));
```

New measurement: 24.20 million, median of 6. 1.01x the previous value.
